# exie1122/micro-quad-SLAM

Measured on NVIDIA B200. Metric: ray_cell_updates_per_s, higher is better.
Workload: dtype i8

## Files before the change

micro-quad-slam_b200/csrc/uqs_api.cu:

```cuda
#include <algorithm>
#include <cmath>
#include <cstdarg>
#include <cstdio>
#include <cstring>
#include <vector>

#include "../../include/uqs_mapping.h"
#include "uqs_host.h"

namespace uqs {

static Context g_single;
Context* g_cur = &g_single;

static char g_err[512] = "";

void set_error(const char* fmt, ...) {
  va_list ap;
  va_start(ap, fmt);
  vsnprintf(g_err, sizeof(g_err), fmt, ap);
  va_end(ap);
}

int cuda_fail(cudaError_t e, const char* what) {
  set_error("CUDA error in %s: %s", what, cudaGetErrorString(e));
  return UQS_ERR_CUDA;
}

int DevBuf::ensure(size_t bytes) {
  if (bytes <= cap) return UQS_OK;
  if (p) cudaFree(p);
  p = nullptr;
  cap = 0;
  size_t want = bytes + bytes / 8 + 256;
  cudaError_t e = cudaMalloc(&p, want);
  if (e != cudaSuccess) {
    cudaGetLastError();
    want = bytes;
    e = cudaMalloc(&p, want);
  }
  if (e != cudaSuccess) {
    p = nullptr;
    set_error("cudaMalloc(%zu) failed: %s", want, cudaGetErrorString(e));
    return UQS_ERR_NOMEM;
  }
  cap = want;
  return UQS_OK;
}

void DevBuf::release() {
  if (p) cudaFree(p);
  p = nullptr;
  cap = 0;
}

int check_ready() {
  if (!g_ctx.ready) {
    if (!g_err[0]) set_error("uqs_init() has not been called or failed");
    return UQS_ERR_NOT_INIT;
  }
  return UQS_OK;
}

int make_dev_params(const uqs_params* p, DevParams* d) {
  if (!p) { set_error("params is NULL"); return UQS_ERR_BAD_ARG; }
  if (p->W < 2 || p->H < 2 || p->W > 32766 || p->H > 32766) {
    set_error("grid size %dx%d outside [2, 32766]", p->W, p->H);
    return UQS_ERR_BAD_ARG;
  }
  if (!(p->res_m > 0.0f) || !std::isfinite(p->origin_x) || !std::isfinite(p->origin_y)) {
    set_error("res_m must be > 0 and the origin finite");
    return UQS_ERR_BAD_ARG;
  }
  if (p->lo_min < -128 || p->lo_max > 127 || p->lo_min > p->lo_max) {
    set_error("log-odds clamp [%d,%d] does not fit int8", p->lo_min, p->lo_max);
    return UQS_ERR_BAD_ARG;
  }
  if (p->lo_free < 0 || p->lo_free > 127 || p->lo_occ < 0 || p->lo_occ > 127) {
    set_error("log-odds steps must be in [0,127]");
    return UQS_ERR_BAD_ARG;
  }
  d->W = p->W; d->H = p->H; d->halfW = p->W / 2; d->halfH = p->H / 2;
  d->res = p->res_m; d->ox = p->origin_x; d->oy = p->origin_y;
  d->max_range = p->max_range_m; d->min_range = p->min_range_m;
  volatile float mr = p->max_range_m, hm = p->hit_margin_m, fov = p->fov_deg;
  volatile float pi_f = (float)M_PI;
  d->hit_below = mr - hm;
  d->half_fov = fov * 0.5f;
  d->deg2rad = pi_f / 180.0f;
  for (int c = 0; c < 8; c++) {
    volatile float cf = (float)c;
    volatile float u = (cf - 3.5f) / 3.5f;
    volatile float hf = d->half_fov;
    d->col_off[c] = u * hf;
  }
  d->lo_free = p->lo_free; d->lo_occ = p->lo_occ; d->lo_min = p->lo_min; d->lo_max = p->lo_max;
  d->end_nohit = -(p->lo_free / 2);
  d->ranges_u16 = 0;
  return UQS_OK;
}

int ensure_inv_table() {
  if (g_ctx.inv_table.p) return UQS_OK;
  std::vector<uint32_t> t(kMaxRayCells + 1);
  t[0] = 0;
  for (uint32_t m = 1; m <= (uint32_t)kMaxRayCells; m++) t[m] = (uint32_t)(((1ull << 31) + m - 1) / m);
  int rc = g_ctx.inv_table.ensure(t.size() * sizeof(uint32_t));
  if (rc) return rc;
  cudaError_t e = cudaMemcpyAsync(g_ctx.inv_table.p, t.data(), t.size() * sizeof(uint32_t), cudaMemcpyHostToDevice, g_ctx.stream());
  if (e == cudaSuccess) e = cudaStreamSynchronize(g_ctx.stream());
  if (e == cudaSuccess) e = cudaDeviceSynchronize();
  if (e != cudaSuccess) { g_ctx.inv_table.release(); return cuda_fail(e, "inv table upload"); }
  return UQS_OK;
}

static void choose_tiles(int W, int rows, int target, int* sw, int* sh, int* nsx, int* nsy) {
  auto pick = [](int extent, int forced, int target, int* size, int* count) {
    if (forced > 0) {
      *size = std::min(forced, extent);
    } else {
      int n = std::max(1, (extent + target / 2) / target);
      int s = (extent + n - 1) / n;
      s = (s + 3) & ~3;
      *size = std::min(s, extent);
    }
    *count = (extent + *size - 1) / *size;
  };
  pick(W, g_ctx.tune_sw, target, sw, nsx);
  pick(rows, g_ctx.tune_sh, target >= 80 ? target + target / 4 : target, sh, nsy);
}

static cudaError_t zero_counted(void* p, size_t bytes, cudaStream_t st) {
  g_ctx.launches += bytes ? 1 : 0;
  return zero_async(p, bytes, st);
}

int replay_device(const DevParams& dp, int n_flights, int n_frames, const float* x, const float* y,
                  const float* yaw, const float* ranges, const uint8_t* kind, int8_t* grids,
                  int accumulate, int row0, int rows, bool reset_stats, const ProbeSet* probes) {
  cudaStream_t st = g_ctx.stream();
  const int gpf = (n_frames + 31) / 32;
  g_ctx.w->boxes_valid = false;
  {
    const int rc0 = ensure_inv_table();
    if (rc0) return rc0;
  }
  {
    const int side = std::max(dp.W, dp.H);
    const bool long_rays = side > kMaxRayCells + 1 && (kind != nullptr || !(dp.max_range / dp.res + 3.0f <= (float)kMaxRayCells));
    bool generic = g_ctx.engine == 3 || long_rays || dp.lo_min > 0 || dp.lo_max < 0;
    int rcg;
    if ((rcg = g_ctx.w->counters.ensure(64 * sizeof(unsigned long long)))) return rcg;
    unsigned long long* cnt = (unsigned long long*)g_ctx.w->counters.p;
    cudaError_t eg = cudaSuccess;
    if (!generic && accumulate) {
      unsigned long long bad = 0;
      eg = zero_counted(cnt + 40, sizeof(unsigned long long), st);
      if (eg == cudaSuccess) eg = range_check_launch(grids, n_flights, dp.W, dp.H, row0, rows, dp.lo_min, dp.lo_max, cnt + 40, st);
      if (eg == cudaSuccess) eg = cudaMemcpyAsync(&bad, cnt + 40, sizeof(bad), cudaMemcpyDeviceToHost, st);
      if (eg == cudaSuccess) eg = cudaStreamSynchronize(st);
      if (eg != cudaSuccess) return cuda_fail(eg, "start-grid range check");
      g_ctx.launches += 1;
      generic = bad != 0;
    }
    if (generic) {
      if (reset_stats) eg = zero_counted(cnt, 8 * sizeof(unsigned long long), st);
      if (eg != cudaSuccess) return cuda_fail(eg, "memset stats");
      ProbeArgs PA;
      if (probes && (rcg = probe_buckets(*probes, 0, n_flights, n_frames, dp.W, 0, 0, 0, 0, 0, 0, &PA))) return rcg;
      KernelTimer t_rep(2);
      eg = generic_launch(dp, n_flights, n_frames, x, y, yaw, ranges, kind, grids, accumulate, row0, rows, cnt, st, probes ? &PA : nullptr);
      t_rep.stop();
      if (eg != cudaSuccess) return cuda_fail(eg, "k_replay_generic launch");
      g_ctx.launches += accumulate ? 1 : 2;
      return UQS_OK;
    }
  }
  int sw, sh, nsx, nsy, slices = 1;
  choose_tiles(dp.W, rows, 80, &sw, &sh, &nsx, &nsy);
  {
    const long long warp_slots = (long long)g_ctx.sm_count * 32;
    const long long jobs80 = (long long)n_flights * nsx * nsy;
    int want = g_ctx.tune_slices;
    int slice_tile = 40;
    const bool band = rows < dp.H;
    if (want == 0 && band && g_ctx.tune_sw == 0 && g_ctx.tune_sh == 0 && jobs80 < 2 * warp_slots) {
      choose_tiles(dp.W, rows, 56, &sw, &sh, &nsx, &nsy);
      want = 1;
    }
    if (want == 0 && jobs80 < 2 * warp_slots) {
      const int s_max = std::max(1, std::min(64, gpf / 8));
      const bool long_rays = dp.max_range >= 200.0f * dp.res;
      long long jobs_t = 1;
      for (int t : { 56, 40, 24, 16 }) {
        if (t == 56 && !long_rays) continue;
        int a, b, nx, ny;
        choose_tiles(dp.W, rows, t, &a, &b, &nx, &ny);
        slice_tile = t;
        jobs_t = (long long)n_flights * nx * ny;
        if (jobs_t * s_max >= 8 * warp_slots) break;
      }
      want = (int)std::min<long long>(s_max, std::max<long long>(1, (16 * warp_slots + jobs_t - 1) / jobs_t));
    }
    if (want > 1) {
      const size_t map_bytes = (size_t)dp.W * dp.H * 4;
      const size_t cap = ((size_t)6 << 30) / map_bytes;
      want = (int)std::min<size_t>((size_t)want, std::max<size_t>(cap, 1) + 1);
    }
    if (want > 1) {
      slices = want;
      choose_tiles(dp.W, rows, slice_tile, &sw, &sh, &nsx, &nsy);
    }
  }
  int pitch = (sw + 3) & ~3;
  if (((pitch >> 2) & 1) == 0) pitch += 4;
  const int pitch_cells = sw | 1;
  if (slices > 1 && g_ctx.tune_slices == 0 && ((size_t)pitch_cells * sh * 4 + kReplayQueueBytes) * kReplayWarps > 227u * 1024u)
    slices = 1;
  const int gps = (gpf + slices - 1) / slices;
  const int tile_bytes = slices > 1 ? std::max(pitch * sh, pitch_cells * sh * 4) : pitch * sh;
  size_t smem = (size_t)tile_bytes * kReplayWarps + (size_t)kReplayQueueBytes * kReplayWarps;

  const int nw = g_ctx.flight_warps ? g_ctx.flight_warps
                 : ((n_flights >= 4 * g_ctx.sm_count || g_ctx.chip_shared) ? 4 : (n_flights >= 2 * g_ctx.sm_count ? 8 : 16));
  const bool may_reside = g_ctx.engine != 1 && row0 == 0 && rows == dp.H;
  if (g_ctx.engine == 2 && !may_reside) {
    set_error("engine 2 (resident) cannot replay a row band");
    return UQS_ERR_BAD_ARG;
  }
  if (smem > 227u * 1024u) {
    set_error("sub-tile %dx%d needs %zu B of shared memory per CTA (> 227 KB)", sw, sh, smem);
    return UQS_ERR_BAD_ARG;
  }

  const size_t per_flight = (size_t)n_frames * (32 * sizeof(uint2) + sizeof(uint4)) + (size_t)gpf * sizeof(uint2);
  const size_t budget = g_ctx.scratch_budget;
  int chunk = (int)std::max<size_t>(1, std::min<size_t>((size_t)n_flights, budget / std::max<size_t>(per_flight, 1)));
  chunk = std::min(chunk, 65535);
  int rc;
  if ((rc = g_ctx.w->rays.ensure((size_t)chunk * n_frames * 32 * sizeof(uint2)))) return rc;
  if ((rc = g_ctx.w->frames.ensure((size_t)chunk * n_frames * sizeof(uint4)))) return rc;
  if ((rc = g_ctx.w->groups.ensure((size_t)chunk * gpf * sizeof(uint2)))) return rc;
  if ((rc = g_ctx.w->counters.ensure(64 * sizeof(unsigned long long)))) return rc;
  unsigned long long* counters = (unsigned long long*)g_ctx.w->counters.p;
  cudaError_t e;
  if (reset_stats) {
    e = zero_counted(counters, 8 * sizeof(unsigned long long), st);
    if (e != cudaSuccess) return cuda_fail(e, "memset stats");
  }

  int ctas_per_sm = 0;
  e = tiles_prepare(probes != nullptr, smem, &ctas_per_sm);
  if (e != cudaSuccess) return cuda_fail(e, "occupancy(k_replay_tiles)");
  if (ctas_per_sm < 1) { set_error("replay kernel does not fit on an SM (smem %zu)", smem); return UQS_ERR_CUDA; }

  for (int f0 = 0; f0 < n_flights; f0 += chunk) {
    const int nf = std::min(chunk, n_flights - f0);
    const size_t fo = (size_t)f0 * n_frames;
    KernelTimer t_setup(1);
    k_ray_setup<<<dim3((unsigned)gpf, (unsigned)nf), 1024, 0, st>>>(
        dp, n_frames, x + fo, y + fo, yaw + fo,
        dp.ranges_u16 ? reinterpret_cast<const float*>(reinterpret_cast<const uint16_t*>(ranges) + fo * 32) : ranges + fo * 32,
        kind ? kind + fo : nullptr, may_reside ? 1 + g_ctx.k0_bias : 0,
        (const uint32_t*)g_ctx.inv_table.p, (uint4*)g_ctx.w->frames.p, (uint2*)g_ctx.w->groups.p, (uint2*)g_ctx.w->rays.p, counters);
    e = cudaGetLastError();
    t_setup.stop();
    if (e != cudaSuccess) return cuda_fail(e, "k_ray_setup launch");

    if (may_reside) {
      if ((rc = g_ctx.w->boxes.ensure((size_t)nf * sizeof(int4)))) return rc;
      int* d_dims = (int*)(counters + 32);
      if (!g_ctx.w->h_dims) {
        e = cudaHostAlloc((void**)&g_ctx.w->h_dims, 16, cudaHostAllocMapped);
        if (e != cudaSuccess) { g_ctx.w->h_dims = nullptr; return cuda_fail(e, "cudaHostAlloc(dims)"); }
      }
      int* h_dims_dev = nullptr;
      e = cudaHostGetDevicePointer((void**)&h_dims_dev, g_ctx.w->h_dims, 0);
      if (e == cudaSuccess) e = zero_counted(d_dims, 2 * sizeof(int), st);
      if (e == cudaSuccess)
        e = flight_boxes_launch(nf, gpf, (const uint2*)g_ctx.w->groups.p, dp.W, dp.H, (int4*)g_ctx.w->boxes.p, d_dims, h_dims_dev, st);
      if (e == cudaSuccess) e = cudaStreamSynchronize(st);
      if (e != cudaSuccess) return cuda_fail(e, "k_flight_boxes");
      const int dims[2] = { g_ctx.w->h_dims[0], g_ctx.w->h_dims[1] };
      g_ctx.launches += 2;
      g_ctx.w->boxes_valid = nf == n_flights;
      g_ctx.w->boxes_n = nf; g_ctx.w->box_w = dims[0]; g_ctx.w->box_h = dims[1];
      const int bw = std::max(dims[0], 4), bh = std::max(dims[1], 1);
      int fpitch = (bw + 3) & ~3;
      if (((fpitch >> 2) & 1) == 0) fpitch += 4;
      if (g_ctx.pitch_mod >= 0)
        while (((fpitch >> 2) & 31) != g_ctx.pitch_mod) fpitch += 4;
      const size_t region = (size_t)fpitch * bh;
      int ring_size = 256, f_ctas = 0, fnw = nw;
      size_t fsmem = 0;
      auto fit = [&](int w, int* ring, size_t* bytes, int* ctas) -> cudaError_t {
        *ring = 256;
        const size_t dec_bytes = (size_t)std::min(w, kDecSlotsMax) * kDecSlotBytes + 16;
        while (*ring > 32 && region + (size_t)(*ring + 4) * w + dec_bytes > kFlightSmemMax) *ring >>= 1;
        *bytes = region + (size_t)(*ring + 4) * w + dec_bytes;
        *ctas = 0;
        return *bytes <= kFlightSmemMax ? flights_prepare(w, g_ctx.flight_fan, g_ctx.flight_prod, *bytes, ctas) : cudaSuccess;
      };
      if (g_ctx.flight_warps) {
        e = fit(fnw, &ring_size, &fsmem, &f_ctas);
      } else {
        e = cudaSuccess;
        for (int w : { 4, 8, 16 }) {
          if (w < nw) continue;
          int r, c;
          size_t bts;
          if ((e = fit(w, &r, &bts, &c)) != cudaSuccess) break;
          if (c < 1) break;
          fnw = w; ring_size = r; fsmem = bts; f_ctas = c;
          if (c * w >= 24) break;
        }
      }
      if (e != cudaSuccess) return cuda_fail(e, "k_replay_flights attributes");
      if (g_ctx.engine == 2 && f_ctas < 1) {
        set_error("engine 2: the touched region %dx%d of a flight does not fit %zu B of shared memory", bw, bh, kFlightSmemMax);
        return UQS_ERR_BAD_ARG;
      }
      const bool pipelined = g_ctx.chip_shared;
      const bool resident = f_ctas >= 1 && (g_ctx.engine == 2 || nf * 4 >= g_ctx.sm_count || pipelined);
      if (resident) {
        FlightArgs FA;
        FA.frames = (const uint4*)g_ctx.w->frames.p;
        FA.rays = (const uint2*)g_ctx.w->rays.p;
        FA.boxes = (const int4*)g_ctx.w->boxes.p;
        FA.grids = grids + (size_t)f0 * dp.W * dp.H;
        FA.job_counter = counters + 8;
        FA.n_flights = nf; FA.n_frames = n_frames;
        FA.W = dp.W; FA.H = dp.H; FA.pitch = fpitch; FA.max_rows = bh; FA.ring_size = ring_size;
        FA.lo_free = dp.lo_free; FA.lo_occ = dp.lo_occ; FA.lo_min = dp.lo_min; FA.lo_max = dp.lo_max;
        FA.end_nohit = dp.end_nohit;
        FA.accumulate = accumulate;
        e = zero_counted(FA.job_counter, sizeof(unsigned long long), st);
        if (e == cudaSuccess && !accumulate) e = zero_counted(FA.grids, (size_t)nf * dp.W * dp.H, st);
        if (e != cudaSuccess) return cuda_fail(e, "memset before k_replay_flights");
        if (probes) {
          int p_ctas = 0;
          ProbeArgs PA;
          if ((rc = probe_buckets(*probes, f0, nf, n_frames, dp.W, 0, 0, 0, 0, 0, 0, &PA))) return rc;
          if ((e = flights_probe_prepare(fnw, fsmem, &p_ctas)) != cudaSuccess) return cuda_fail(e, "k_replay_flights (probes) attributes");
          if (p_ctas < 1) { set_error("resident engine (probes): %zu B of shared memory do not fit an SM", fsmem); return UQS_ERR_CUDA; }
          KernelTimer t_rep(2);
          e = flights_probe_launch(fnw, (unsigned)std::min<long long>(nf, (long long)p_ctas * g_ctx.sm_count), fsmem, st, FA, PA);
          t_rep.stop();
          if (e != cudaSuccess) return cuda_fail(e, "k_replay_flights (probes) launch");
          g_ctx.launches += 2;
          continue;
        }
        const unsigned fgrid = (unsigned)std::min<long long>(nf, (long long)f_ctas * g_ctx.sm_count);
        KernelTimer t_rep(2);
        e = flights_launch(fnw, g_ctx.flight_fan, g_ctx.flight_prod, fgrid, fsmem, st, FA);
        t_rep.stop();
        if (e != cudaSuccess) return cuda_fail(e, "k_replay_flights launch");
        g_ctx.launches += 2;
        continue;
      }
    }
    if (g_ctx.w->order_nsx != nsx || g_ctx.w->order_nsy != nsy) {
      std::vector<uint32_t> ord((size_t)nsx * nsy);
      for (uint32_t i = 0; i < ord.size(); i++) ord[i] = i;
      auto dist2 = [&](uint32_t t) {
        const double cx = ((t % nsx) + 0.5) * sw - dp.W * 0.5, cy = ((t / nsx) + 0.5) * sh + row0 - dp.H * 0.5;
        return cx * cx + cy * cy;
      };
      std::stable_sort(ord.begin(), ord.end(), [&](uint32_t a, uint32_t b) { return dist2(a) < dist2(b); });
      if ((rc = g_ctx.w->order.ensure(ord.size() * sizeof(uint32_t)))) return rc;
      e = cudaMemcpyAsync(g_ctx.w->order.p, ord.data(), ord.size() * sizeof(uint32_t), cudaMemcpyHostToDevice, st);
      if (e == cudaSuccess) e = cudaStreamSynchronize(st);
      if (e != cudaSuccess) return cuda_fail(e, "tile order upload");
      g_ctx.w->order_nsx = nsx;
      g_ctx.w->order_nsy = nsy;
    }
    ReplayArgs A;
    A.tile_order = (const uint32_t*)g_ctx.w->order.p;
    A.n_flights = nf;
    A.frames = (const uint4*)g_ctx.w->frames.p;
    A.groups = (const uint2*)g_ctx.w->groups.p;
    A.rays = (const uint2*)g_ctx.w->rays.p;
    A.grids = grids + (size_t)f0 * dp.W * dp.H;
    A.job_counter = counters + 8;
    A.total_jobs = (unsigned long long)nf * nsx * nsy * slices;
    A.slices = slices; A.groups_per_slice = gps; A.pitch_cells = pitch_cells;
    A.maps = nullptr;
    if (slices > 1) {
      if ((rc = g_ctx.w->maps.ensure((size_t)nf * (slices - 1) * dp.W * dp.H * sizeof(uint32_t)))) return rc;
      A.maps = (uint32_t*)g_ctx.w->maps.p;
    }
    A.n_frames = n_frames; A.groups_per_flight = gpf;
    A.W = dp.W; A.H = dp.H; A.row0 = row0; A.rows = rows;
    A.sw = sw; A.sh = sh; A.nsx = nsx; A.nsy = nsy;
    A.pitch = pitch; A.tile_bytes = tile_bytes;
    A.lo_free = dp.lo_free; A.lo_occ = dp.lo_occ; A.lo_min = dp.lo_min; A.lo_max = dp.lo_max;
    A.end_nohit = dp.end_nohit;
    A.accumulate = accumulate;
    e = zero_counted(A.job_counter, sizeof(unsigned long long), st);
    if (e != cudaSuccess) return cuda_fail(e, "memset job counter");
    unsigned long long want = (A.total_jobs + kReplayWarps - 1) / kReplayWarps;
    unsigned grid = (unsigned)std::min<unsigned long long>(want, (unsigned long long)ctas_per_sm * g_ctx.sm_count);
    ProbeArgs PA;
    if (probes && (rc = probe_buckets(*probes, f0, nf, n_frames, dp.W, slices, gps, sw, sh, nsx, nsy, &PA))) return rc;
    KernelTimer t_rep(2);
    e = tiles_launch(probes != nullptr, grid, smem, st, A, probes ? PA : ProbeArgs{});
    if (e == cudaSuccess && probes && slices > 1 &&
        (rc = probe_resolve_slices(PA, (int)probes->slots(), A.grids, A.maps, dp.W, dp.H, slices, gps)))
      return rc;
    if (e == cudaSuccess && slices > 1) {
      const size_t cells = (size_t)dp.W * rows * nf;
      k_compose_slices<<<(unsigned)((cells + 255) / 256), 256, 0, st>>>(A.grids, A.maps, nf, dp.W, dp.H, slices, row0, rows);
      e = cudaGetLastError();
      g_ctx.launches += 1;
    }
    t_rep.stop();
    if (e != cudaSuccess) return cuda_fail(e, "k_replay_tiles launch");
    g_ctx.launches += 2;
  }
  return UQS_OK;
}

int fetch_stats_mask(uqs_stats* stats, uint64_t frames, unsigned mask) {
  if (!stats) return UQS_OK;
  unsigned long long tot[4] = { 0, 0, 0, 0 };
  for (int i = 0; i < 3; i++) {
    if (!(mask & (1u << i)) || !g_ctx.works[i].counters.p) continue;
    Work* saved = g_ctx.w;
    g_ctx.w = &g_ctx.works[i];
    cudaStream_t st = g_ctx.stream();
    g_ctx.w = saved;
    unsigned long long h[4];
    cudaError_t e = cudaMemcpyAsync(h, g_ctx.works[i].counters.p, sizeof(h), cudaMemcpyDeviceToHost, st);
    if (e != cudaSuccess) return cuda_fail(e, "stats D2H");
    e = cudaStreamSynchronize(st);
    if (e != cudaSuccess) return cuda_fail(e, "stats sync");
    for (int k = 0; k < 4; k++) tot[k] += h[k];
  }
  stats->ray_cell_updates = tot[0];
  stats->rays_accepted = tot[1];
  stats->rays_skipped = tot[2];
  stats->domain_errors = tot[3];
  stats->frames = frames;
  if (tot[3]) {
    set_error("%llu rays longer than %d cells reached a fast engine (internal routing error)", tot[3], kMaxRayCells);
    return UQS_ERR_DOMAIN;
  }
  return UQS_OK;
}

int fetch_stats(uqs_stats* stats, uint64_t frames) { return fetch_stats_mask(stats, frames, 1u); }

int pose_device(int n_flights, int n_samples, const uint32_t* t_ms, const float* rx, const float* ry,
                const float* h, const float* yaw, const uint8_t* q, float* xo, float* yo, int mode) {
  cudaStream_t st = g_ctx.stream();
  const long long total = (long long)n_flights * n_samples;
  int rc;
  if ((rc = g_ctx.w->inc.ensure((size_t)total * 2 * sizeof(float)))) return rc;
  if ((rc = g_ctx.w->counters.ensure(64 * sizeof(unsigned long long)))) return rc;
  float* inc_n = (float*)g_ctx.w->inc.p;
  float* inc_e = inc_n + total;
  unsigned long long* dom = nullptr;
  cudaError_t e = cudaSuccess;
  volatile float pi_f = (float)M_PI;
  const float deg2rad = pi_f / 180.0f;
  KernelTimer t_pose(0);
  k_pose_increments<<<(unsigned)((total + 255) / 256), 256, 0, st>>>(total, n_samples, t_ms, rx, ry, h, yaw, q,
                                                                     deg2rad, inc_n, inc_e, dom);
  e = cudaGetLastError();
  if (e != cudaSuccess) return cuda_fail(e, "k_pose_increments launch");
  if (mode == 0) {
    const int warps_per_block = 4;
    k_pose_chain<<<(unsigned)((n_flights + warps_per_block - 1) / warps_per_block), warps_per_block * 32, 0, st>>>(
        n_flights, n_samples, inc_n, inc_e, xo, yo);
  } else {
    const int tile = pose_scan_tile();
    const int ppf = (n_samples + tile - 1) / tile;
    const size_t nparts = (size_t)n_flights * ppf;
    if ((rc = g_ctx.w->scan.ensure(nparts * pose_scan_state_bytes() + 64))) return rc;
    e = cudaMemsetAsync(g_ctx.w->scan.p, 0, nparts * pose_scan_state_bytes() + 64, st);
    if (e != cudaSuccess) return cuda_fail(e, "memset scan state");
    unsigned int* ticket = (unsigned int*)((char*)g_ctx.w->scan.p + nparts * pose_scan_state_bytes());
    k_pose_scan<<<(unsigned)nparts, pose_scan_threads(), 0, st>>>(n_flights, n_samples, ppf, inc_n, inc_e, xo, yo,
                                                                  (volatile ScanState*)g_ctx.w->scan.p, ticket);
  }
  e = cudaGetLastError();
  t_pose.stop();
  if (e != cudaSuccess) return cuda_fail(e, "pose kernel launch");
  g_ctx.launches += 2;
  return UQS_OK;
}

void context_select_single() {
  g_cur = &g_single;
  if (g_single.ready) cudaSetDevice(g_single.device);
}

int context_init(Context& c, int device) {
  int n = 0;
  cudaError_t e = cudaGetDeviceCount(&n);
  if (e != cudaSuccess || n <= 0) {
    cudaGetLastError();
    set_error("no CUDA device available (%s); this library has no CPU fallback",
              e != cudaSuccess ? cudaGetErrorString(e) : "device count is 0");
    c.ready = false;
    return UQS_ERR_NO_DEVICE;
  }
  if (device < 0 || device >= n) { set_error("device %d out of range (0..%d)", device, n - 1); return UQS_ERR_BAD_ARG; }
  if ((e = cudaSetDevice(device)) != cudaSuccess) return cuda_fail(e, "cudaSetDevice");
  cudaDeviceProp prop;
  if ((e = cudaGetDeviceProperties(&prop, device)) != cudaSuccess) return cuda_fail(e, "cudaGetDeviceProperties");
  if (prop.major < 10) {
    set_error("device %d is sm_%d%d; this library is built for sm_100a only", device, prop.major, prop.minor);
    return UQS_ERR_NO_DEVICE;
  }
  if ((e = cudaStreamCreateWithFlags(&c.own_stream, cudaStreamNonBlocking)) != cudaSuccess)
    return cuda_fail(e, "cudaStreamCreate");
  c.device = device;
  c.sm_count = prop.multiProcessorCount;
  c.ext_stream = nullptr;
  c.use_ext = false;
  c.ready = true;
  g_err[0] = 0;
  return UQS_OK;
}

void context_shutdown(Context& c) {
  if (!c.ready) return;
  cudaSetDevice(c.device);
  cudaDeviceSynchronize();
  comm_release();
  dropin_release();
  pipeline_release();
  c.release_all();
  if (c.own_stream) cudaStreamDestroy(c.own_stream);
  c.own_stream = nullptr;
  c.ready = false;
}

}

using namespace uqs;

extern "C" {

void uqs_params_default(uqs_params* p) {
  if (!p) return;
  p->W = 500; p->H = 500; p->res_m = 0.10f; p->size_m = 50.0f;
  p->origin_x = 0.0f; p->origin_y = 0.0f;
  p->max_range_m = 4.00f; p->fov_deg = 63.0f;
  p->min_range_m = 0.05f; p->hit_margin_m = 0.05f;
  p->lo_free = 1; p->lo_occ = 6; p->lo_min = -80; p->lo_max = 80;
}

const char* uqs_last_error(void) { return g_err; }

int uqs_init(int device) {
  g_cur = &g_single;
  if (g_single.ready && g_single.device == device) {
    cudaSetDevice(device);
    return UQS_OK;
  }
  if (g_single.ready) uqs_shutdown();
  return context_init(g_single, device);
}

void uqs_shutdown(void) {
  Context* saved = g_cur;
  g_cur = &g_single;
  context_shutdown(g_single);
  g_cur = (saved == &g_single) ? &g_single : saved;
}

int uqs_device_sm_count(void) { return g_ctx.ready ? g_ctx.sm_count : 0; }

int uqs_set_stream(void* s) {
  int rc = check_ready();
  if (rc) return rc;
  g_ctx.ext_stream = (cudaStream_t)s;
  g_ctx.use_ext = true;
  return UQS_OK;
}

int uqs_use_own_stream(void) {
  int rc = check_ready();
  if (rc) return rc;
  g_ctx.use_ext = false;
  return UQS_OK;
}

int uqs_sync(void) {
  int rc = check_ready();
  if (rc) return rc;
  cudaError_t e = cudaStreamSynchronize(g_ctx.stream());
  if (e != cudaSuccess) return cuda_fail(e, "cudaStreamSynchronize");
  return UQS_OK;
}

int uqs_set_tuning(int sw, int sh, int time_slices) {
  if (sw < 0 || sh < 0 || time_slices < 0) { set_error("negative tuning value"); return UQS_ERR_BAD_ARG; }
  g_ctx.tune_sw = sw;
  g_ctx.tune_sh = sh;
  g_ctx.tune_slices = time_slices;
  return UQS_OK;
}

int uqs_set_engine(int engine, int flight_warps) {
  if (engine < 0 || engine > 3 || (flight_warps != 0 && flight_warps != 4 && flight_warps != 8 && flight_warps != 16 && flight_warps != 32)) {
    set_error("engine must be 0 (auto), 1 (sub-tiles), 2 (grid resident) or 3 (unrestricted); warps 0, 4, 8, 16 or 32");
    return UQS_ERR_BAD_ARG;
  }
  g_ctx.engine = engine;
  g_ctx.flight_warps = flight_warps;
  return UQS_OK;
}

int uqs_set_resident_pitch_mod(int words_mod32) {
  g_ctx.pitch_mod = words_mod32 < 0 ? -1 : (words_mod32 & 31);
  return UQS_OK;
}

int uqs_set_decode_warp(int on) {
  g_ctx.flight_prod = on < 0 ? kDefaultDecodeWarp : (on ? 1 : 0);
  return UQS_OK;
}

int uqs_set_k0_bias(int steps) {
  g_ctx.k0_bias = steps < 0 ? 0 : (steps > 8 ? 8 : steps);
  return UQS_OK;
}

int uqs_set_fan_layout(int on) {
  g_ctx.flight_fan = on < 0 ? kDefaultFanLayout : (on ? 1 : 0);
  return UQS_OK;
}

unsigned long long uqs_kernel_launches(void) { return g_ctx.launches; }

int uqs_set_profiling(int on) {
  int rc = check_ready();
  if (rc) return rc;
  g_ctx.profiling = on != 0;
  return UQS_OK;
}

int uqs_profile_collect(double ms[3], int counts[3]) {
  int rc = check_ready();
  if (rc) return rc;
  cudaError_t e = cudaStreamSynchronize(g_ctx.stream());
  if (e != cudaSuccess) return cuda_fail(e, "profile sync");
  for (int i = 0; i < 3; i++) { ms[i] = 0.0; counts[i] = 0; }
  for (auto& s : g_ctx.spans) {
    float t = 0.f;
    if (s.kind < 3 && cudaEventElapsedTime(&t, s.a, s.b) == cudaSuccess) { ms[s.kind] += t; counts[s.kind]++; }
    cudaEventDestroy(s.a);
    cudaEventDestroy(s.b);
  }
  g_ctx.spans.clear();
  return UQS_OK;
}

int uqs_profile_timeline(double* out, int max_spans) {
  int rc = check_ready();
  if (rc) return -1;
  if (cudaDeviceSynchronize() != cudaSuccess || g_ctx.spans.empty() || !out) return 0;
  int n = 0;
  const cudaEvent_t ref = g_ctx.spans[0].a;
  for (auto& s : g_ctx.spans) {
    if (n >= max_spans) break;
    float t0 = 0.f, t1 = 0.f;
    if (cudaEventElapsedTime(&t0, ref, s.a) != cudaSuccess || cudaEventElapsedTime(&t1, ref, s.b) != cudaSuccess) continue;
    out[3 * n] = s.kind; out[3 * n + 1] = t0; out[3 * n + 2] = t1;
    n++;
  }
  return n;
}

int uqs_replay_dev(const uqs_params* p, int n_flights, int n_frames, const float* x, const float* y,
                   const float* yaw, const float* ranges, int8_t* grids, int accumulate, int row0,
                   int rows, uqs_stats* stats) {
  int rc = check_ready();
  if (rc) return rc;
  DevParams dp;
  if ((rc = make_dev_params(p, &dp))) return rc;
  if (n_flights <= 0 || n_frames <= 0 || !x || !y || !yaw || !ranges || !grids) {
    set_error("uqs_replay_dev: NULL pointer or non-positive size");
    return UQS_ERR_BAD_ARG;
  }
  if (row0 < 0 || rows <= 0 || row0 + rows > p->H) { set_error("row range [%d,%d) outside the grid", row0, row0 + rows); return UQS_ERR_BAD_ARG; }
  if ((rc = replay_device(dp, n_flights, n_frames, x, y, yaw, ranges, nullptr, grids, accumulate, row0, rows, true)))
    return rc;
  return fetch_stats(stats, (uint64_t)n_flights * n_frames);
}

int uqs_pose_integrate_dev(int n_flights, int n_samples, const uint32_t* t_ms, const float* rx,
                           const float* ry, const float* h, const float* yaw, const uint8_t* q,
                           float* xo, float* yo, int mode) {
  int rc = check_ready();
  if (rc) return rc;
  if (n_flights <= 0 || n_samples <= 0 || !t_ms || !rx || !ry || !h || !yaw || !q || !xo || !yo || (mode != 0 && mode != 1)) {
    set_error("uqs_pose_integrate_dev: bad argument");
    return UQS_ERR_BAD_ARG;
  }
  return pose_device(n_flights, n_samples, t_ms, rx, ry, h, yaw, q, xo, yo, mode);
}


static int h2d(DevBuf& b, const void* src, size_t bytes, const char* what) {
  int rc = b.ensure(bytes);
  if (rc) return rc;
  cudaError_t e = cudaMemcpyAsync(b.p, src, bytes, cudaMemcpyHostToDevice, g_ctx.stream());
  if (e != cudaSuccess) return cuda_fail(e, what);
  return UQS_OK;
}

int uqs_pose_integrate(int n_flights, int n_samples, const uint32_t* t_ms, const float* rx,
                       const float* ry, const float* h, const float* yaw, const uint8_t* q,
                       float* xo, float* yo, int mode) {
  int rc = check_ready();
  if (rc) return rc;
  if (n_flights <= 0 || n_samples <= 0 || !t_ms || !rx || !ry || !h || !yaw || !q || !xo || !yo || (mode != 0 && mode != 1)) {
    set_error("uqs_pose_integrate: bad argument");
    return UQS_ERR_BAD_ARG;
  }
  const size_t n = (size_t)n_flights * n_samples;
  if ((rc = h2d(g_ctx.in_t, t_ms, n * 4, "t_ms H2D"))) return rc;
  if ((rc = h2d(g_ctx.in_rx, rx, n * 4, "of_rate_x H2D"))) return rc;
  if ((rc = h2d(g_ctx.in_ry, ry, n * 4, "of_rate_y H2D"))) return rc;
  if ((rc = h2d(g_ctx.in_h, h, n * 4, "h_m H2D"))) return rc;
  if ((rc = h2d(g_ctx.in_yaw, yaw, n * 4, "yaw H2D"))) return rc;
  if ((rc = h2d(g_ctx.in_q, q, n, "of_q H2D"))) return rc;
  if ((rc = g_ctx.in_x.ensure(n * 4)) || (rc = g_ctx.in_y.ensure(n * 4))) return rc;
  if ((rc = pose_device(n_flights, n_samples, (uint32_t*)g_ctx.in_t.p, (float*)g_ctx.in_rx.p, (float*)g_ctx.in_ry.p,
                        (float*)g_ctx.in_h.p, (float*)g_ctx.in_yaw.p, (uint8_t*)g_ctx.in_q.p, (float*)g_ctx.in_x.p,
                        (float*)g_ctx.in_y.p, mode)))
    return rc;
  cudaError_t e = cudaMemcpyAsync(xo, g_ctx.in_x.p, n * 4, cudaMemcpyDeviceToHost, g_ctx.stream());
  if (e == cudaSuccess) e = cudaMemcpyAsync(yo, g_ctx.in_y.p, n * 4, cudaMemcpyDeviceToHost, g_ctx.stream());
  if (e == cudaSuccess) e = cudaStreamSynchronize(g_ctx.stream());
  if (e != cudaSuccess) return cuda_fail(e, "pose D2H");
  return UQS_OK;
}

int uqs_beam_cells(const uqs_params* p, int n_frames, const float* x, const float* y, const float* yaw,
                   const float* ranges, int32_t* cells_out, int32_t* origin_out) {
  int rc = check_ready();
  if (rc) return rc;
  DevParams dp;
  if ((rc = make_dev_params(p, &dp))) return rc;
  if (n_frames <= 0 || !x || !y || !yaw || !ranges || !cells_out || !origin_out) { set_error("uqs_beam_cells: bad argument"); return UQS_ERR_BAD_ARG; }
  if ((rc = ensure_inv_table())) return rc;
  cudaStream_t st = g_ctx.stream();
  const size_t n = (size_t)n_frames;
  const int gpf = (n_frames + 31) / 32;
  if ((rc = h2d(g_ctx.in_x, x, n * 4, "x H2D")) || (rc = h2d(g_ctx.in_y, y, n * 4, "y H2D")) ||
      (rc = h2d(g_ctx.in_yaw, yaw, n * 4, "yaw H2D")) || (rc = h2d(g_ctx.in_ranges, ranges, n * 128, "ranges H2D")))
    return rc;
  if ((rc = g_ctx.w->rays.ensure(n * 32 * sizeof(uint2))) || (rc = g_ctx.w->frames.ensure(n * sizeof(uint4))) ||
      (rc = g_ctx.w->groups.ensure((size_t)gpf * sizeof(uint2))) || (rc = g_ctx.w->counters.ensure(64 * 8)) ||
      (rc = g_ctx.out_grids.ensure(n * 32 * 2 * 4 + n * 2 * 4)))
    return rc;
  cudaError_t e = cudaMemsetAsync(g_ctx.w->counters.p, 0, 64, st);
  if (e != cudaSuccess) return cuda_fail(e, "memset");
  k_ray_setup<<<(unsigned)gpf, 1024, 0, st>>>(dp, n_frames, (float*)g_ctx.in_x.p, (float*)g_ctx.in_y.p,
                                              (float*)g_ctx.in_yaw.p, (float*)g_ctx.in_ranges.p, nullptr, 0,
                                              (const uint32_t*)g_ctx.inv_table.p, (uint4*)g_ctx.w->frames.p, (uint2*)g_ctx.w->groups.p,
                                              (uint2*)g_ctx.w->rays.p, (unsigned long long*)g_ctx.w->counters.p);
  int32_t* d_cells = (int32_t*)g_ctx.out_grids.p;
  int32_t* d_origin = d_cells + n * 64;
  k_records_to_cells<<<(unsigned)((n * 32 + 255) / 256), 256, 0, st>>>((long long)n, (uint4*)g_ctx.w->frames.p,
                                                                       (uint2*)g_ctx.w->rays.p, d_cells, d_origin);
  e = cudaGetLastError();
  if (e != cudaSuccess) return cuda_fail(e, "beam_cells kernels");
  e = cudaMemcpyAsync(cells_out, d_cells, n * 64 * 4, cudaMemcpyDeviceToHost, st);
  if (e == cudaSuccess) e = cudaMemcpyAsync(origin_out, d_origin, n * 2 * 4, cudaMemcpyDeviceToHost, st);
  if (e == cudaSuccess) e = cudaStreamSynchronize(st);
  if (e != cudaSuccess) return cuda_fail(e, "beam_cells D2H");
  g_ctx.launches += 2;
  return UQS_OK;
}

int uqs_frame_bounds(const uqs_params* p, int n_frames, const float* x, const float* y, const float* yaw,
                     const float* ranges, int32_t* k0_out, int32_t* sorted_out) {
  int rc = check_ready();
  if (rc) return rc;
  DevParams dp;
  if ((rc = make_dev_params(p, &dp))) return rc;
  if (n_frames <= 0 || !x || !y || !yaw || !ranges || !k0_out || !sorted_out) { set_error("uqs_frame_bounds: bad argument"); return UQS_ERR_BAD_ARG; }
  if ((rc = ensure_inv_table())) return rc;
  cudaStream_t st = g_ctx.stream();
  const size_t n = (size_t)n_frames;
  const int gpf = (n_frames + 31) / 32;
  if ((rc = h2d(g_ctx.in_x, x, n * 4, "x H2D")) || (rc = h2d(g_ctx.in_y, y, n * 4, "y H2D")) ||
      (rc = h2d(g_ctx.in_yaw, yaw, n * 4, "yaw H2D")) || (rc = h2d(g_ctx.in_ranges, ranges, n * 128, "ranges H2D")))
    return rc;
  if ((rc = g_ctx.w->rays.ensure(n * 32 * sizeof(uint2))) || (rc = g_ctx.w->frames.ensure(n * sizeof(uint4))) ||
      (rc = g_ctx.w->groups.ensure((size_t)gpf * sizeof(uint2))) || (rc = g_ctx.w->counters.ensure(64 * 8)))
    return rc;
  cudaError_t e = cudaMemsetAsync(g_ctx.w->counters.p, 0, 64, st);
  if (e != cudaSuccess) return cuda_fail(e, "memset");
  k_ray_setup<<<(unsigned)gpf, 1024, 0, st>>>(dp, n_frames, (float*)g_ctx.in_x.p, (float*)g_ctx.in_y.p,
                                              (float*)g_ctx.in_yaw.p, (float*)g_ctx.in_ranges.p, nullptr, 1,
                                              (const uint32_t*)g_ctx.inv_table.p, (uint4*)g_ctx.w->frames.p, (uint2*)g_ctx.w->groups.p,
                                              (uint2*)g_ctx.w->rays.p, (unsigned long long*)g_ctx.w->counters.p);
  e = cudaGetLastError();
  if (e != cudaSuccess) return cuda_fail(e, "k_ray_setup launch");
  std::vector<uint4> fr(n);
  e = cudaMemcpyAsync(fr.data(), g_ctx.w->frames.p, n * sizeof(uint4), cudaMemcpyDeviceToHost, st);
  if (e == cudaSuccess) e = cudaStreamSynchronize(st);
  if (e != cudaSuccess) return cuda_fail(e, "frame_bounds D2H");
  for (size_t i = 0; i < n; i++) {
    k0_out[i] = (fr[i].y & kFrameHasOrigin) ? (int32_t)(fr[i].x >> 16) : -1;
    sorted_out[i] = (fr[i].y & kFrameSorted) ? 1 : 0;
  }
  g_ctx.launches += 1;
  return UQS_OK;
}

int uqs_sincosf_batch(size_t n, const float* ang, float* s, float* c) {
  int rc = check_ready();
  if (rc) return rc;
  if (!n || !ang || !s || !c) { set_error("uqs_sincosf_batch: bad argument"); return UQS_ERR_BAD_ARG; }
  cudaStream_t st = g_ctx.stream();
  if ((rc = h2d(g_ctx.in_x, ang, n * 4, "ang H2D")) || (rc = g_ctx.in_y.ensure(n * 4)) || (rc = g_ctx.in_yaw.ensure(n * 4)))
    return rc;
  k_sincosf<<<(unsigned)((n + 255) / 256), 256, 0, st>>>(n, (float*)g_ctx.in_x.p, (float*)g_ctx.in_y.p, (float*)g_ctx.in_yaw.p);
  cudaError_t e = cudaGetLastError();
  if (e == cudaSuccess) e = cudaMemcpyAsync(s, g_ctx.in_y.p, n * 4, cudaMemcpyDeviceToHost, st);
  if (e == cudaSuccess) e = cudaMemcpyAsync(c, g_ctx.in_yaw.p, n * 4, cudaMemcpyDeviceToHost, st);
  if (e == cudaSuccess) e = cudaStreamSynchronize(st);
  if (e != cudaSuccess) return cuda_fail(e, "sincosf batch");
  g_ctx.launches += 1;
  return UQS_OK;
}

int uqs_measure_rmw_peak(double* updates_per_s) {
  int rc = check_ready();
  if (rc) return rc;
  if (!updates_per_s) { set_error("NULL output"); return UQS_ERR_BAD_ARG; }
  cudaStream_t st = g_ctx.stream();
  const int tile_bytes = 4096, iters = 8192;
  const size_t smem = (size_t)tile_bytes * kReplayWarps;
  cudaError_t e = cudaFuncSetAttribute(k_rmw_peak, cudaFuncAttributeMaxDynamicSharedMemorySize, (int)smem);
  if (e != cudaSuccess) return cuda_fail(e, "cudaFuncSetAttribute(k_rmw_peak)");
  int per_sm = 0;
  e = cudaOccupancyMaxActiveBlocksPerMultiprocessor(&per_sm, k_rmw_peak, kReplayThreads, smem);
  if (e != cudaSuccess || per_sm < 1) return cuda_fail(e, "occupancy(k_rmw_peak)");
  if ((rc = g_ctx.w->counters.ensure(64 * 8))) return rc;
  const unsigned grid = (unsigned)(per_sm * g_ctx.sm_count);
  cudaEvent_t a, b;
  cudaEventCreate(&a);
  cudaEventCreate(&b);
  k_rmw_peak<<<grid, kReplayThreads, smem, st>>>(tile_bytes, 64, -80, (int*)g_ctx.w->counters.p + 96);
  cudaEventRecord(a, st);
  k_rmw_peak<<<grid, kReplayThreads, smem, st>>>(tile_bytes, iters, -80, (int*)g_ctx.w->counters.p + 96);
  cudaEventRecord(b, st);
  e = cudaEventSynchronize(b);
  float ms = 0.f;
  cudaEventElapsedTime(&ms, a, b);
  cudaEventDestroy(a);
  cudaEventDestroy(b);
  if (e != cudaSuccess) return cuda_fail(e, "k_rmw_peak");
  const double updates = (double)grid * kReplayThreads * (double)iters * 8.0;
  *updates_per_s = updates / (ms * 1e-3);
  g_ctx.launches += 2;
  return UQS_OK;
}

int uqs_measure_atoms_peak(double* updates_per_s) {
  int rc = check_ready();
  if (rc) return rc;
  if (!updates_per_s) { set_error("NULL output"); return UQS_ERR_BAD_ARG; }
  cudaStream_t st = g_ctx.stream();
  const int tile_bytes = 4096, iters = 2048;
  const size_t smem = (size_t)tile_bytes * kReplayWarps;
  cudaError_t e = cudaFuncSetAttribute(k_atoms_peak, cudaFuncAttributeMaxDynamicSharedMemorySize, (int)smem);
  if (e != cudaSuccess) return cuda_fail(e, "cudaFuncSetAttribute(k_atoms_peak)");
  int per_sm = 0;
  e = cudaOccupancyMaxActiveBlocksPerMultiprocessor(&per_sm, k_atoms_peak, kReplayThreads, smem);
  if (e != cudaSuccess || per_sm < 1) return cuda_fail(e, "occupancy(k_atoms_peak)");
  if ((rc = g_ctx.w->counters.ensure(64 * 8))) return rc;
  const unsigned grid = (unsigned)(per_sm * g_ctx.sm_count);
  cudaEvent_t a, b;
  cudaEventCreate(&a);
  cudaEventCreate(&b);
  k_atoms_peak<<<grid, kReplayThreads, smem, st>>>(tile_bytes, 64, (int*)g_ctx.w->counters.p + 96);
  cudaEventRecord(a, st);
  k_atoms_peak<<<grid, kReplayThreads, smem, st>>>(tile_bytes, iters, (int*)g_ctx.w->counters.p + 96);
  cudaEventRecord(b, st);
  e = cudaEventSynchronize(b);
  float ms = 0.f;
  cudaEventElapsedTime(&ms, a, b);
  cudaEventDestroy(a);
  cudaEventDestroy(b);
  if (e != cudaSuccess) return cuda_fail(e, "k_atoms_peak");
  *updates_per_s = (double)grid * kReplayThreads * (double)iters * 8.0 / (ms * 1e-3);
  g_ctx.launches += 2;
  return UQS_OK;
}

}
```

micro-quad-slam_b200/csrc/uqs_device.cuh:

```cuda
#pragma once
#include <cstdint>
#include <cuda_runtime.h>

namespace uqs {

struct DevParams {
  int   W, H, halfW, halfH;
  float res, ox, oy;
  float max_range, min_range, hit_below;
  float half_fov;
  float col_off[8];
  float deg2rad;
  int   lo_free, lo_occ, lo_min, lo_max;
  int   end_nohit;
  int   ranges_u16;
};

__device__ __forceinline__ float range_from_mm(unsigned mm) {
  return mm == 0xFFFFu ? __int_as_float(0x7fc00000) : __fmul_rn((float)mm, 0.001f);
}

constexpr int      kMaxRayCells   = 1024;
constexpr uint32_t kRayHit        = 1u << 24;
constexpr uint32_t kRayValid      = 1u << 25;
constexpr uint32_t kFrameHasOrigin = 1u << 16;
constexpr uint32_t kFrameSorted    = 1u << 17;
constexpr uint32_t kEmptyBoxLoHi  = 0x00007fffu;

static __constant__ uint32_t kInvPio4[24] = {
  0xa2, 0xa2f9, 0xa2f983, 0xa2f9836e, 0xf9836e4e, 0x836e4e44, 0x6e4e4415, 0x4e441529, 0x441529fc, 0x1529fc27,
  0x29fc2757, 0xfc2757d1, 0x2757d1f5, 0x57d1f534, 0xd1f534dd, 0xf534ddc0, 0x34ddc0db, 0xddc0db62, 0xc0db6295,
  0xdb629599, 0x6295993c, 0x95993c43, 0x993c4390, 0x3c439041 };

__device__ __forceinline__ void sincosf_poly(double x, double xs, bool swap, bool neg_cos, float& sn, float& cs) {
  const double x2 = __dmul_rn(x, x);
  const double x3 = __dmul_rn(x2, xs);
  const double x4 = __dmul_rn(x2, x2);
  const double s1 = __fma_rn(x2, -0x1.994eb3774cf24p-13, 0x1.1107605230bc4p-7);
  const double c2 = __fma_rn(x2, 0x1.99343027bf8c3p-16, -0x1.6c087e89a359dp-10);
  const double c1 = __fma_rn(x2, -0x1.ffffffd0c621cp-2, 1.0);
  const double x5 = __dmul_rn(x2, x3);
  const double x6 = __dmul_rn(x2, x4);
  double S = __fma_rn(x3, -0x1.555545995a603p-3, xs);
  double C = __fma_rn(x4, 0x1.55553e1068f19p-5, c1);
  S = __fma_rn(x5, s1, S);
  C = __fma_rn(x6, c2, C);
  if (neg_cos) C = -C;
  const float fs = __double2float_rn(S), fc = __double2float_rn(C);
  if (swap) { cs = fs; sn = fc; } else { sn = fs; cs = fc; }
}

static __device__ __noinline__ void sincosf_large(float y, float& sn, float& cs) {
  uint32_t xi = __float_as_uint(y);
  if (((xi >> 20) & 0x7ffu) >= 0x7f8u) {
    const uint32_t nan = ((xi & 0x7fffffffu) == 0x7f800000u) ? 0xffc00000u : (xi | 0x00400000u);
    sn = cs = __uint_as_float(nan);
    return;
  }
  const int sign = (int)(xi >> 31);
  const uint32_t* arr = &kInvPio4[(xi >> 26) & 15u];
  const int shift = (int)((xi >> 23) & 7u);
  xi = ((xi & 0xffffffu) | 0x800000u) << shift;
  unsigned long long res0 = (unsigned long long)(uint32_t)(xi * arr[0]);
  const unsigned long long res1 = (unsigned long long)xi * arr[4];
  const unsigned long long res2 = (unsigned long long)xi * arr[8];
  res0 = (res2 >> 32) | (res0 << 32);
  res0 += res1;
  const unsigned long long nn = (res0 + (1ull << 61)) >> 62;
  res0 -= nn << 62;
  const double x = __dmul_rn(__ll2double_rn((long long)res0), 0x1.921FB54442D18p-62);
  const int n = (int)nn;
  const double xs = (((n + sign) + 1) & 2) ? -x : x;
  sincosf_poly(x, xs, (n & 1) != 0, ((n + sign) & 2) != 0, sn, cs);
}

__device__ __forceinline__ bool sincosf_glibc(float y, float& sn, float& cs) {
  const uint32_t top12 = (__float_as_uint(y) >> 20) & 0x7ffu;
  if (top12 >= 0x42fu) {
    sincosf_large(y, sn, cs);
    return true;
  }
  double x = (double)y;
  const double r = __dmul_rn(x, 0x1.45f306dc9c883p+23);
  const int n = (__double2int_rz(r) + 0x800000) >> 24;
  x = __fma_rn(-(double)n, 0x1.921fb54442d18p+0, x);
  const double xs = ((n + 1) & 2) ? -x : x;
  const double x2 = __dmul_rn(x, x);
  const double x3 = __dmul_rn(x2, xs);
  const double x4 = __dmul_rn(x2, x2);
  const double s1 = __fma_rn(x2, -0x1.994eb3774cf24p-13, 0x1.1107605230bc4p-7);
  const double c2 = __fma_rn(x2, 0x1.99343027bf8c3p-16, -0x1.6c087e89a359dp-10);
  const double c1 = __fma_rn(x2, -0x1.ffffffd0c621cp-2, 1.0);
  const double x5 = __dmul_rn(x2, x3);
  const double x6 = __dmul_rn(x2, x4);
  double S = __fma_rn(x3, -0x1.555545995a603p-3, xs);
  double C = __fma_rn(x4, 0x1.55553e1068f19p-5, c1);
  S = __fma_rn(x5, s1, S);
  C = __fma_rn(x6, c2, C);
  if (n & 2) C = -C;
  const float fs = __double2float_rn(S), fc = __double2float_rn(C);
  const bool tiny = top12 < 0x398u;
  if (n & 1) { cs = fs; sn = fc; } else { sn = fs; cs = fc; }
  if (tiny) { sn = y; cs = 1.0f; }
  return true;
}

__device__ __forceinline__ int lrintf_as_int(float q) {
  if (fabsf(q) < 2147483520.0f) return __float2int_rn(q);
  const long long r = (fabsf(q) < 9223372036854775808.0f) ? __float2ll_rn(q)
                                                          : (long long)0x8000000000000000ull;
  return (int)r;
}

__device__ __forceinline__ bool world_to_grid(const DevParams& p, float wx, float wy, int& gx,
                                              int& gy) {
  const float ddx = __fsub_rn(wx, p.ox);
  const float ddy = __fsub_rn(wy, p.oy);
  const int ix = (int)((unsigned)lrintf_as_int(__fdiv_rn(ddx, p.res)) + (unsigned)p.halfW);
  const int iy = (int)((unsigned)lrintf_as_int(__fdiv_rn(ddy, p.res)) + (unsigned)p.halfH);
  gx = ix;
  gy = iy;
  return !(ix < 0 || ix >= p.W || iy < 0 || iy >= p.H);
}

__device__ __forceinline__ int beam_endpoint(const DevParams& p, float px, float py, float yaw_deg,
                                             float dist, int b, float& ex, float& ey, bool& hit) {
  if (isnan(dist)) return 0;
  if (dist <= p.min_range) return 0;
  hit = dist < p.hit_below;
  if (dist > p.max_range) dist = p.max_range;
  const int d = b >> 3, c = b & 7;
  const float centre = (d & 1) ? ((d & 2) ? -90.0f : 90.0f) : ((d & 2) ? 180.0f : 0.0f);
  const float off = p.col_off[c];
  const float ang_deg = __fadd_rn(__fadd_rn(yaw_deg, centre), off);
  const float ang = __fmul_rn(ang_deg, p.deg2rad);
  float sn, cs;
  if (!sincosf_glibc(ang, sn, cs)) return -1;
  ex = __fadd_rn(px, __fmul_rn(dist, cs));
  ey = __fadd_rn(py, __fmul_rn(dist, sn));
  return 1;
}

__device__ __forceinline__ int sext12(uint32_t v) { return ((int)(v << 20)) >> 20; }

__device__ __forceinline__ float frontier_ray_angle(const DevParams& p, float yaw_deg, float offset_deg, int r) {
  const float ro = (r == 0) ? 0.0f : (r == 1) ? 15.0f : -15.0f;
  return __fmul_rn(__fadd_rn(__fadd_rn(yaw_deg, offset_deg), ro), p.deg2rad);
}
__device__ __forceinline__ float frontier_step(const DevParams& p) { return __fmul_rn(p.res, 2.0f); }
constexpr float kFrontierRange = 2.5f;
__device__ __forceinline__ bool frontier_point(const DevParams& p, float x, float y, float d, float ca, float sa, int& gx,
                                               int& gy) {
  const float px = __fadd_rn(x, __fmul_rn(d, ca));
  const float py = __fadd_rn(y, __fmul_rn(d, sa));
  return world_to_grid(p, px, py, gx, gy);
}
__device__ __forceinline__ int frontier_weight(int v) {
  return (v >= -1 && v <= 1) ? 3 : (v > 10) ? -4 : (v < -10) ? 1 : 0;
}

__device__ __forceinline__ int minor_steps(int k, int n2, int h2, uint32_t inv) {
  return (int)__umulhi((uint32_t)(k * n2 + h2), inv);
}

}
```

micro-quad-slam_b200/csrc/uqs_host.h:

```cpp
#pragma once
#include <cstddef>
#include <cstdint>
#include <cuda_runtime.h>
#include <vector>

#include "../../include/uqs_mapping.h"
#include "uqs_kernels.cuh"

namespace uqs {

constexpr int kDefaultDecodeWarp = 0;
constexpr int kDefaultFanLayout = 0;

struct DevBuf {
  void* p = nullptr;
  size_t cap = 0;
  int ensure(size_t bytes);
  void release();
};

struct Work {
  DevBuf rays, frames, groups, counters, inc, scan, order, maps, boxes;
  DevBuf probe_slots, probe_keys, probe_sorted, probe_start, probe_tmp;
  int order_nsx = 0, order_nsy = 0;
  cudaStream_t stream = nullptr;
  int* h_dims = nullptr;
  bool boxes_valid = false;
  int boxes_n = 0, box_w = 0, box_h = 0;
  void release() {
    if (h_dims) cudaFreeHost(h_dims);
    h_dims = nullptr;
    DevBuf* all[] = { &rays, &frames, &groups, &counters, &inc, &scan, &order, &maps, &boxes, &probe_slots, &probe_keys, &probe_sorted,
                      &probe_start, &probe_tmp };
    order_nsx = order_nsy = 0;
    for (DevBuf* b : all) b->release();
  }
};

struct Context {
  bool ready = false;
  int device = -1;
  int sm_count = 0;
  cudaStream_t own_stream = nullptr;
  cudaStream_t ext_stream = nullptr;
  bool use_ext = false;
  int tune_sw = 0, tune_sh = 0, tune_slices = 0;
  int engine = 0;
  int flight_warps = 0;
  int k0_bias = 0;
  int pitch_mod = -1;
  int flight_prod = kDefaultDecodeWarp;
  int flight_fan = kDefaultFanLayout;
  int host_chunk = 0;
  bool copy_only = false;
  bool chip_shared = false;
  size_t scratch_budget = (size_t)12 << 30;
  unsigned long long launches = 0;
  DevBuf inv_table;
  Work works[3];
  Work* w = &works[0];
  DevBuf in_t, in_rx, in_ry, in_h, in_yaw, in_q, in_x, in_y, in_ranges, in_kind, out_grids;
  void* pipeline = nullptr;
  void* comm = nullptr;
  int comm_rank = 0, comm_nranks = 1;
  int band_edges[17] = { 0 };

  bool profiling = false;
  struct Span { cudaEvent_t a, b; int kind; };
  std::vector<Span> spans;

  cudaStream_t stream() const { return w->stream ? w->stream : (use_ext ? ext_stream : own_stream); }
  cudaStream_t user_stream() const { return use_ext ? ext_stream : own_stream; }
  void release_all() {
    DevBuf* all[] = { &in_t, &in_rx, &in_ry, &in_h, &in_yaw, &in_q, &in_x, &in_y, &in_ranges, &in_kind, &out_grids };
    for (DevBuf* b : all) b->release();
    for (Work& k : works) k.release();
    inv_table.release();
  }
};

constexpr size_t kFlightSmemMax = 227u * 1024u - 64u;

extern Context* g_cur;
#define g_ctx (*::uqs::g_cur)
int context_init(Context& c, int device);
void context_shutdown(Context& c);
void context_select_single();

void set_error(const char* fmt, ...);
int cuda_fail(cudaError_t e, const char* what);
int check_ready();
int make_dev_params(const uqs_params* p, DevParams* d);
struct ProbeSet {
  int n_queries = 0, s_max = 0;
  const uqs_query* queries = nullptr;
  const int* cells = nullptr;
  uint32_t* values = nullptr;
  size_t slots() const { return (size_t)n_queries * 3 * s_max; }
};
int probe_buckets(const ProbeSet& Q, int f0, int nf, int n_frames, int W, int slices, int groups_per_slice, int sw,
                  int sh, int nsx, int nsy, ProbeArgs* out);
int probe_resolve_slices(const ProbeArgs& A, int n_probes_max, const int8_t* grids, const uint32_t* maps, int W, int H,
                         int slices, int groups_per_slice);

int replay_device(const DevParams& dp, int n_flights, int n_frames, const float* x, const float* y,
                  const float* yaw, const float* ranges, const uint8_t* kind, int8_t* grids,
                  int accumulate, int row0, int rows, bool reset_stats, const ProbeSet* probes = nullptr);
int fetch_stats(uqs_stats* stats, uint64_t frames);
int ensure_inv_table();
cudaError_t generic_launch(const DevParams& dp, int n_flights, int n_frames, const float* x, const float* y, const float* yaw,
                           const float* ranges, const uint8_t* kind, int8_t* grids, int accumulate, int row0, int rows,
                           unsigned long long* stats, cudaStream_t st, const ProbeArgs* Q = nullptr);
cudaError_t range_check_launch(const int8_t* grids, int n_flights, int W, int H, int row0, int rows, int lo_min, int lo_max,
                               unsigned long long* bad, cudaStream_t st);
int fetch_stats_mask(uqs_stats* stats, uint64_t frames, unsigned mask);
void dropin_release();
void pipeline_release();
void comm_release();
int pose_device(int n_flights, int n_samples, const uint32_t* t_ms, const float* rx, const float* ry,
                const float* h, const float* yaw, const uint8_t* q, float* xo, float* yo, int mode);

struct KernelTimer {
  int kind;
  cudaStream_t st;
  cudaEvent_t a = nullptr, b = nullptr;
  explicit KernelTimer(int k, cudaStream_t on = nullptr) : kind(k), st(on ? on : g_ctx.stream()) {
    if (g_ctx.profiling && cudaEventCreate(&a) == cudaSuccess && cudaEventCreate(&b) == cudaSuccess)
      cudaEventRecord(a, st);
  }
  void stop() {
    if (a && b) {
      cudaEventRecord(b, st);
      g_ctx.spans.push_back({a, b, kind});
    }
  }
};

}
```

micro-quad-slam_b200/csrc/uqs_kernels.cu:

```cuda
#include <algorithm>
#include <cstdio>

#include "uqs_kernels.cuh"

namespace uqs {


__global__ void k_pose_increments(long long total, int n_samples, const uint32_t* __restrict__ t_ms,
                                  const float* __restrict__ rate_x, const float* __restrict__ rate_y,
                                  const float* __restrict__ h_m, const float* __restrict__ yaw_deg,
                                  const uint8_t* __restrict__ q, float deg2rad,
                                  float* __restrict__ inc_n, float* __restrict__ inc_e,
                                  unsigned long long* __restrict__ ) {
  const long long i = (long long)blockIdx.x * blockDim.x + threadIdx.x;
  if (i >= total) return;
  const int s = (int)(i % n_samples);
  float dn = 0.0f, de = 0.0f;
  if (s > 0) {
    const float rx = rate_x[i], ry = rate_y[i], h = h_m[i], yw = yaw_deg[i];
    if (q[i] >= 50 && !isnan(rx) && !isnan(ry) && !isnan(h) && !isnan(yw)) {
      const float dt = __fmul_rn((float)(t_ms[i] - t_ms[i - 1]), 0.001f);
      const float vbx = __fmul_rn(rx, h);
      const float vby = __fmul_rn(ry, h);
      const float a = __fmul_rn(yw, deg2rad);
      float sn, cs;
      sincosf_glibc(a, sn, cs);
      const float vn = __fsub_rn(__fmul_rn(vbx, cs), __fmul_rn(vby, sn));
      const float ve = __fadd_rn(__fmul_rn(vbx, sn), __fmul_rn(vby, cs));
      dn = __fmul_rn(vn, dt);
      de = __fmul_rn(ve, dt);
    }
  }
  inc_n[i] = dn;
  inc_e[i] = de;
}

constexpr int kChainChunk = 256;
constexpr int kChainWarps = 4;

__global__ void __launch_bounds__(kChainWarps * 32)
k_pose_chain(int n_flights, int n_samples, const float* __restrict__ inc_n,
             const float* __restrict__ inc_e, float* __restrict__ xo,
             float* __restrict__ yo) {
  __shared__ __align__(16) float s_n[kChainWarps][kChainChunk], s_e[kChainWarps][kChainChunk];
  const int wib = threadIdx.x >> 5, lane = threadIdx.x & 31;
  const int flight = blockIdx.x * kChainWarps + wib;
  if (flight >= n_flights) return;
  const size_t base = (size_t)flight * n_samples;
  float* sn = s_n[wib];
  float* se = s_e[wib];
  constexpr int PER = kChainChunk / 32;
  float rn[PER], re[PER];
  auto fetch = [&](int s0) {
#pragma unroll
    for (int u = 0; u < PER; u++) {
      const int s = s0 + u * 32 + lane;
      rn[u] = (s < n_samples) ? __ldg(&inc_n[base + s]) : 0.0f;
      re[u] = (s < n_samples) ? __ldg(&inc_e[base + s]) : 0.0f;
    }
  };
  fetch(0);
  float px = 0.0f, py = 0.0f;
  for (int s0 = 0; s0 < n_samples; s0 += kChainChunk) {
#pragma unroll
    for (int u = 0; u < PER; u++) { sn[u * 32 + lane] = rn[u]; se[u * 32 + lane] = re[u]; }
    if (s0 + kChainChunk < n_samples) fetch(s0 + kChainChunk);
    __syncwarp();
    if (lane == 0) {
      const float4* vn = reinterpret_cast<const float4*>(sn);
      const float4* ve = reinterpret_cast<const float4*>(se);
      float4 a0 = vn[0], b0 = ve[0], a1 = vn[1], b1 = ve[1];
#pragma unroll 4
      for (int g = 0; g < kChainChunk / 4; g++) {
        const int gn = min(g + 2, kChainChunk / 4 - 1);
        const float4 a2 = vn[gn], b2 = ve[gn];
        float4 a = a0, b = b0;
        a.x = px = __fadd_rn(px, a.x); b.x = py = __fadd_rn(py, b.x);
        a.y = px = __fadd_rn(px, a.y); b.y = py = __fadd_rn(py, b.y);
        a.z = px = __fadd_rn(px, a.z); b.z = py = __fadd_rn(py, b.z);
        a.w = px = __fadd_rn(px, a.w); b.w = py = __fadd_rn(py, b.w);
        reinterpret_cast<float4*>(sn)[g] = a;
        reinterpret_cast<float4*>(se)[g] = b;
        a0 = a1; b0 = b1; a1 = a2; b1 = b2;
      }
    }
    __syncwarp();
#pragma unroll
    for (int u = 0; u < PER; u++) {
      const int s = s0 + u * 32 + lane;
      if (s < n_samples) { xo[base + s] = sn[u * 32 + lane]; yo[base + s] = se[u * 32 + lane]; }
    }
    __syncwarp();
  }
}

constexpr int kScanThreads = 256;
constexpr int kScanItems = 8;
constexpr int kScanTile = kScanThreads * kScanItems;

struct ScanState { double agg_n, agg_e, inc_n, inc_e; int flag; int pad; };

__global__ void __launch_bounds__(kScanThreads)
k_pose_scan(int n_flights, int n_samples, int parts_per_flight, const float* __restrict__ inc_n,
            const float* __restrict__ inc_e, float* __restrict__ xo, float* __restrict__ yo,
            volatile ScanState* state, unsigned int* ticket) {
  __shared__ unsigned int s_part;
  __shared__ double s_wn[kScanThreads / 32], s_we[kScanThreads / 32];
  __shared__ double s_prefix_n, s_prefix_e;
  if (threadIdx.x == 0) s_part = atomicAdd(ticket, 1u);
  __syncthreads();
  const unsigned int part = s_part;
  if (part >= (unsigned)(n_flights * parts_per_flight)) return;
  const int flight = part / parts_per_flight, pf = part % parts_per_flight;
  const size_t base = (size_t)flight * n_samples;
  const int s_begin = pf * kScanTile + threadIdx.x * kScanItems;

  double vn[kScanItems], ve[kScanItems];
  double tn = 0.0, te = 0.0;
#pragma unroll
  for (int k = 0; k < kScanItems; k++) {
    const int s = s_begin + k;
    const double a = (s < n_samples) ? (double)inc_n[base + s] : 0.0;
    const double b = (s < n_samples) ? (double)inc_e[base + s] : 0.0;
    tn += a; te += b;
    vn[k] = tn; ve[k] = te;
  }
  const int lane = threadIdx.x & 31, wid = threadIdx.x >> 5;
  double wn = tn, we = te;
#pragma unroll
  for (int o = 1; o < 32; o <<= 1) {
    const double un = __shfl_up_sync(0xffffffffu, wn, o), ue = __shfl_up_sync(0xffffffffu, we, o);
    if (lane >= o) { wn += un; we += ue; }
  }
  if (lane == 31) { s_wn[wid] = wn; s_we[wid] = we; }
  __syncthreads();
  double off_n = 0.0, off_e = 0.0;
  for (int w = 0; w < wid; w++) { off_n += s_wn[w]; off_e += s_we[w]; }
  const double excl_n = off_n + wn - tn, excl_e = off_e + we - te;

  if (threadIdx.x == kScanThreads - 1) {
    const double agg_n = off_n + wn, agg_e = off_e + we;
    double pre_n = 0.0, pre_e = 0.0;
    if (pf == 0) {
      state[part].inc_n = agg_n; state[part].inc_e = agg_e;
      __threadfence();
      state[part].flag = 2;
    } else {
      state[part].agg_n = agg_n; state[part].agg_e = agg_e;
      __threadfence();
      state[part].flag = 1;
      int p = (int)part - 1;
      for (;;) {
        int f;
        while ((f = state[p].flag) == 0) { }
        __threadfence();
        if (f == 2) { pre_n += state[p].inc_n; pre_e += state[p].inc_e; break; }
        pre_n += state[p].agg_n; pre_e += state[p].agg_e;
        p--;
      }
      state[part].inc_n = pre_n + agg_n; state[part].inc_e = pre_e + agg_e;
      __threadfence();
      state[part].flag = 2;
    }
    s_prefix_n = pre_n; s_prefix_e = pre_e;
  }
  __syncthreads();
  const double bn = s_prefix_n + excl_n, be = s_prefix_e + excl_e;
#pragma unroll
  for (int k = 0; k < kScanItems; k++) {
    const int s = s_begin + k;
    if (s < n_samples) {
      xo[base + s] = (float)(bn + vn[k]);
      yo[base + s] = (float)(be + ve[k]);
    }
  }
}

int pose_scan_tile() { return kScanTile; }
int pose_scan_threads() { return kScanThreads; }
size_t pose_scan_state_bytes() { return sizeof(ScanState); }

__device__ __forceinline__ void mbar_init(uint32_t bar, uint32_t count) {
  asm volatile("mbarrier.init.shared::cta.b64 [%0], %1;" ::"r"(bar), "r"(count) : "memory");
  asm volatile("fence.mbarrier_init.release.cluster;" ::: "memory");
  asm volatile("fence.proxy.async.shared::cta;" ::: "memory");
}
__device__ __forceinline__ void bulk_load_g2s(uint32_t dst, const void* src, uint32_t bytes, uint32_t bar) {
  asm volatile("mbarrier.arrive.expect_tx.shared::cta.b64 _, [%0], %1;" ::"r"(bar), "r"(bytes) : "memory");
  asm volatile("cp.async.bulk.shared::cluster.global.mbarrier::complete_tx::bytes [%0], [%1], %2, [%3];" ::"r"(dst), "l"(src),
               "r"(bytes), "r"(bar)
               : "memory");
}
__device__ __forceinline__ void mbar_wait(uint32_t bar, uint32_t parity) {
  asm volatile(
      "{\n"
      ".reg .pred p;\n"
      "UQS_WAIT:\n"
      "mbarrier.try_wait.parity.shared::cta.b64 p, [%0], %1;\n"
      "@!p bra UQS_WAIT;\n"
      "}\n" ::"r"(bar),
      "r"(parity)
      : "memory");
}

__global__ void __launch_bounds__(1024, 2)
k_ray_setup(const __grid_constant__ DevParams p, int n_frames, const float* __restrict__ x,
            const float* __restrict__ y, const float* __restrict__ yaw_deg,
            const float* __restrict__ ranges, const uint8_t* __restrict__ kind, int want_k0,
            const uint32_t* __restrict__ inv_table, uint4* __restrict__ frames, uint2* __restrict__ groups, uint2* __restrict__ rays,
            unsigned long long* __restrict__ stats ) {
  __shared__ __align__(128) float s_rng[32 * 32];
  __shared__ __align__(8) unsigned long long s_bar;
  __shared__ int s_box[4][32];
  __shared__ unsigned s_cnt[2][32];
  __shared__ int s_org[32][2];
  const int lane = threadIdx.x & 31, w = threadIdx.x >> 5;
  const int flight = blockIdx.y, g = blockIdx.x, groups_per_flight = gridDim.x;
  const int f = g * 32 + w;
  const size_t fbase = (size_t)flight * n_frames;
  const int nfr = min(32, n_frames - g * 32);

  const bool u16 = p.ranges_u16 != 0;
  const unsigned rbytes = u16 ? 64u : 128u;
  const unsigned char* ranges_b = reinterpret_cast<const unsigned char*>(ranges);
  const unsigned char* blk_ranges = ranges_b + (fbase + (size_t)g * 32) * rbytes;
  const bool staged = (reinterpret_cast<size_t>(ranges) & 15) == 0;
  const uint32_t bar_sa = (uint32_t)__cvta_generic_to_shared(&s_bar);
  if (staged) {
    if (threadIdx.x == 0) {
      mbar_init(bar_sa, 1);
      bulk_load_g2s((uint32_t)__cvta_generic_to_shared(s_rng), blk_ranges, (uint32_t)nfr * rbytes, bar_sa);
    }
    __syncthreads();
  }

  int xmin = 0x7fff, xmax = 0, ymin = 0x7fff, ymax = 0;
  unsigned cells = 0;
  int accepted = 0, skipped = 0, domain = 0;

  if (w == 31) {
    int ox = -1, oy = -1;
    const int fo = g * 32 + lane;
    if (fo < n_frames && !world_to_grid(p, x[fbase + fo], y[fbase + fo], ox, oy)) ox = oy = -1;
    s_org[lane][0] = ox;
    s_org[lane][1] = oy;
  }

  const bool live = f < n_frames;
  const size_t fi = fbase + (live ? f : 0);
  float ex = 0.f, ey = 0.f;
  bool hit = false, raw = false;
  int st = 0;
  if (live) {
    const float px = x[fi], py = y[fi], third = yaw_deg[fi];
    raw = kind != nullptr && kind[fi] == 1;
    if (staged) mbar_wait(bar_sa, 0);
    const unsigned char* rb = staged ? reinterpret_cast<const unsigned char*>(s_rng) + (size_t)w * rbytes : ranges_b + fi * rbytes;
    const float* rr = reinterpret_cast<const float*>(rb);
    if (!raw) {
      const float dist = u16 ? range_from_mm(reinterpret_cast<const uint16_t*>(rb)[lane]) : rr[lane];
      st = beam_endpoint(p, px, py, third, dist, lane, ex, ey, hit);
    } else {
      st = (lane == 0) ? 1 : 0;
      ex = third;
      ey = rr[0];
      hit = rr[1] != 0.0f;
    }
  }
  __syncthreads();

  if (live) {
    const int gx0 = s_org[w][0], gy0 = s_org[w][1];
    const bool have_o = gx0 >= 0;
    uint32_t w0 = 0, w1 = 0;
    if (st < 0) {
      domain = 1;
    } else if (st > 0 && have_o) {
      int gx1, gy1;
      if (world_to_grid(p, ex, ey, gx1, gy1)) {
        const int dx = gx1 - gx0, dy = gy1 - gy0;
        const int m = max(abs(dx), abs(dy));
        if (m > kMaxRayCells) {
          domain = 1;
        } else {
          w0 = ((uint32_t)dx & 0xfffu) | (((uint32_t)dy & 0xfffu) << 12) | (hit ? kRayHit : 0u) |
               kRayValid;
          w1 = __ldg(&inv_table[m]);
          xmin = min(gx0, gx1); xmax = max(gx0, gx1);
          ymin = min(gy0, gy1); ymax = max(gy0, gy1);
          cells = (unsigned)m + 1u;
          accepted = 1;
        }
      }
    }
    if (!accepted && !domain && !(raw && lane != 0)) skipped = 1;
    rays[fi * 32 + lane] = make_uint2(w0, w1);

    int k0 = 0;
    bool frame_sorted = false;
    if (want_k0) {
      const int dx = sext12(w0), dy = sext12(w0 >> 12);
      const int adx = abs(dx), ady = abs(dy);
      const bool xmaj = adx >= ady;
      const int m = accepted ? (xmaj ? adx : ady) : -1;
      const int n = xmaj ? ady : adx;
      const bool xpos = dx >= 0, ypos = dy >= 0;
      float ra, rb;
      if (xmaj) { ra = xpos ? (ypos ? 0.f : 8.f) : 4.f; rb = (xpos == ypos) ? 1.f : -1.f; }
      else      { ra = ypos ? 2.f : 6.f;                rb = (xpos == ypos) ? -1.f : 1.f; }
      float sigma = (m > 0) ? ra + rb * __fdividef((float)n, (float)m) : 0.f;
      if (sigma >= 8.f) sigma -= 8.f;
      const int mmax = __reduce_max_sync(0xffffffffu, m);
      const unsigned any = __ballot_sync(0xffffffffu, m >= 0);
      const unsigned dir = __ballot_sync(0xffffffffu, m >= 1);
      const unsigned above = dir & ~(0xffffffffu >> (31 - lane));
      const int nxt = above ? (__ffs(above) - 1) : (__ffs(dir) - 1);
      const float sn = __shfl_sync(0xffffffffu, sigma, nxt & 31);
      const bool has_dir = m >= 1;
      float gap = sn - sigma;
      int A = (int)ra, sgn_n = (rb > 0.f) ? n : -n;
      if (A == 8 && n == 0) A = 0;
      const int pk = (A << 24) | ((sgn_n & 0xfff) << 12) | (max(m, 0) & 0xfff);
      const int pn = __shfl_sync(0xffffffffu, pk, nxt & 31);
      const int A2 = pn >> 24, n2s = (pn << 8) >> 20, m2 = pn & 0xfff;
      const int order = (A2 - A) * m * m2 + n2s * m - sgn_n * m2;
      const bool wraps = has_dir && order < 0;
      if (order == 0) gap = 0.f;
      else if (order < 0) gap += 8.f;
      gap = fmaxf(gap, 0.f);
      const bool sorted = __popc(__ballot_sync(0xffffffffu, wraps)) <= 1;
      frame_sorted = sorted;
      if (__popc(any) >= 2) {
        if (sorted || __popc(dir) < 2) {
          int kk = 1;
          if (has_dir && __popc(dir) >= 2) kk = (gap > 1e-4f) ? (int)(1.0f / (gap - 2e-5f)) + 1 : 0x7fffffff;
          k0 = min(__reduce_max_sync(0xffffffffu, kk) + (want_k0 - 1), mmax + 1);
        } else {
#pragma unroll 4
          for (int j = 1; j <= 16; j++) {
            const int pl = (lane + j) & 31;
            const float sp = __shfl_sync(0xffffffffu, sigma, pl);
            const int mp = __shfl_sync(0xffffffffu, m, pl);
            float dlt = fabsf(sigma - sp);
            dlt = fminf(dlt, 8.f - dlt);
            int kk = (dlt > 1e-4f) ? (int)(1.0f / (dlt - 2e-5f)) + 1 : 0x7fffffff;
            if (m < 1 || mp < 1) kk = 1;
            kk = min(kk, min(m, mp) + 1);
            if (m >= 0 && mp >= 0) k0 = max(k0, kk);
          }
          k0 = __reduce_max_sync(0xffffffffu, k0);
        }
      }
    }

    xmin = __reduce_min_sync(0xffffffffu, xmin);
    xmax = __reduce_max_sync(0xffffffffu, xmax);
    ymin = __reduce_min_sync(0xffffffffu, ymin);
    ymax = __reduce_max_sync(0xffffffffu, ymax);
    if (lane == 0)
      frames[fi] = make_uint4(have_o ? ((uint32_t)gx0 | ((uint32_t)k0 << 16)) : 0u,
                              have_o ? ((uint32_t)gy0 | kFrameHasOrigin | (frame_sorted ? kFrameSorted : 0u)) : 0u,
                              (uint32_t)xmin | ((uint32_t)xmax << 16),
                              (uint32_t)ymin | ((uint32_t)ymax << 16));
  }
  const unsigned as = __reduce_add_sync(0xffffffffu, (unsigned)accepted | ((unsigned)skipped << 16));
  const unsigned cd = __reduce_add_sync(0xffffffffu, cells | ((unsigned)domain << 21));
  if (lane == 0) {
    s_box[0][w] = xmin; s_box[1][w] = xmax; s_box[2][w] = ymin; s_box[3][w] = ymax;
    s_cnt[0][w] = as; s_cnt[1][w] = cd;
  }
  __syncthreads();
  if (w == 0) {
    const int bx0 = __reduce_min_sync(0xffffffffu, s_box[0][lane]);
    const int bx1 = __reduce_max_sync(0xffffffffu, s_box[1][lane]);
    const int by0 = __reduce_min_sync(0xffffffffu, s_box[2][lane]);
    const int by1 = __reduce_max_sync(0xffffffffu, s_box[3][lane]);
    const unsigned bas = __reduce_add_sync(0xffffffffu, s_cnt[0][lane]);
    const unsigned long long bcd = s_cnt[1][lane];
    const unsigned bc = __reduce_add_sync(0xffffffffu, (unsigned)(bcd & 0x1fffffu));
    const unsigned bd = __reduce_add_sync(0xffffffffu, (unsigned)(bcd >> 21));
    if (lane == 0)
      groups[(size_t)flight * groups_per_flight + g] =
          make_uint2((uint32_t)bx0 | ((uint32_t)bx1 << 16), (uint32_t)by0 | ((uint32_t)by1 << 16));
    if (lane < 4) {
      const unsigned long long t = lane == 0 ? bc : (lane == 1 ? (bas & 0xffffu) : (lane == 2 ? (bas >> 16) : bd));
      if (t) atomicAdd(&stats[lane], t);
    }
  }
}

__global__ void k_records_to_cells(long long n_frames, const uint4* __restrict__ frames,
                                   const uint2* __restrict__ rays, int32_t* __restrict__ cells,
                                   int32_t* __restrict__ origin) {
  const long long i = (long long)blockIdx.x * blockDim.x + threadIdx.x;
  if (i >= n_frames * 32) return;
  const long long f = i >> 5;
  const uint4 fr = frames[f];
  const uint2 r = rays[i];
  int cx = -1, cy = -1;
  if (r.x & kRayValid) {
    cx = (int)(fr.x & 0xffffu) + sext12(r.x);
    cy = (int)(fr.y & 0xffffu) + sext12(r.x >> 12);
  }
  cells[2 * i] = cx;
  cells[2 * i + 1] = cy;
  if ((i & 31) == 0) {
    origin[2 * f] = (fr.y & kFrameHasOrigin) ? (int)(fr.x & 0xffffu) : -1;
    origin[2 * f + 1] = (fr.y & kFrameHasOrigin) ? (int)(fr.y & 0xffffu) : -1;
  }
}

__global__ void k_sincosf(size_t n, const float* __restrict__ a, float* __restrict__ s,
                          float* __restrict__ c) {
  const size_t i = (size_t)blockIdx.x * blockDim.x + threadIdx.x;
  if (i >= n) return;
  float sn, cs;
  sincosf_glibc(a[i], sn, cs);
  s[i] = sn;
  c[i] = cs;
}

__global__ void k_world_to_grid_one(DevParams p, float wx, float wy, int* out ) {
  int gx, gy;
  const bool ok = world_to_grid(p, wx, wy, gx, gy);
  out[0] = ok ? 1 : 0;
  out[1] = gx;
  out[2] = gy;
}


__device__ __forceinline__ bool box_overlaps(uint32_t xlohi, uint32_t ylohi, int X0, int X1, int Y0,
                                             int Y1) {
  const int bx0 = (int)(xlohi & 0xffffu), bx1 = (int)(xlohi >> 16);
  const int by0 = (int)(ylohi & 0xffffu), by1 = (int)(ylohi >> 16);
  return bx0 < X1 && bx1 >= X0 && by0 < Y1 && by1 >= Y0;
}

struct SmemRegion { uint32_t lo, hi; };
#ifdef UQS_DEBUG_BOUNDS
__device__ __noinline__ void uqs_bounds_fail(uint32_t a, uint32_t n, uint32_t lo, uint32_t hi, int line) {
  printf("UQS_DEBUG_BOUNDS: shared access [%u, %u) outside region [%u, %u) at uqs_kernels.cu:%d (block %d thread %d)\n", a, a + n,
         lo, hi, line, (int)blockIdx.x, (int)threadIdx.x);
  __trap();
}
#define UQS_CHECK(a, n, R) do { const uint32_t a_ = (a); if (a_ < (R).lo || a_ + (n) > (R).hi) uqs_bounds_fail(a_, (n), (R).lo, (R).hi, __LINE__); } while (0)
#else
#define UQS_CHECK(a, n, R) ((void)0)
#endif

__device__ __forceinline__ int lds_s8(uint32_t a) {
  int v;
  asm volatile("ld.shared.s8 %0, [%1];" : "=r"(v) : "r"(a) : "memory");
  return v;
}
__device__ __forceinline__ void sts_u8(uint32_t a, int v) {
  asm volatile("st.shared.u8 [%0], %1;" ::"r"(a), "r"(v) : "memory");
}
__device__ __forceinline__ uint32_t lds_u32(uint32_t a) {
  uint32_t v;
  asm volatile("ld.shared.u32 %0, [%1];" : "=r"(v) : "r"(a) : "memory");
  return v;
}
__device__ __forceinline__ void sts_u32(uint32_t a, uint32_t v) {
  asm volatile("st.shared.u32 [%0], %1;" ::"r"(a), "r"(v) : "memory");
}
__device__ __forceinline__ uint4 lds_v4(uint32_t a) {
  uint4 v;
  asm volatile("ld.shared.v4.u32 {%0,%1,%2,%3}, [%4];" : "=r"(v.x), "=r"(v.y), "=r"(v.z), "=r"(v.w) : "r"(a) : "memory");
  return v;
}
__device__ __forceinline__ void sts_v4(uint32_t a, uint32_t x, uint32_t y, uint32_t z, uint32_t w) {
  asm volatile("st.shared.v4.u32 [%0], {%1,%2,%3,%4};" ::"r"(a), "r"(x), "r"(y), "r"(z), "r"(w) : "memory");
}
__device__ __forceinline__ int in_reg(int v) {
  asm volatile("" : "+r"(v));
  return v;
}


struct TileConsts { int pitch, lo_free, lo_occ, lo_min, lo_max, end_nohit; };
struct TileRegions { SmemRegion tile, queue; };

__device__ __forceinline__ int div_small(int num, int den) {
  int q = (int)((float)num * __frcp_rn((float)den));
  const int r = num - q * den;
  q += (r >= den) ? 1 : 0;
  q -= (r < 0) ? 1 : 0;
  return q;
}

constexpr int kQueueEntries = 64;
constexpr int kQueueBytes = kQueueEntries * 12;
static_assert(kQueueBytes == kReplayQueueBytes, "the host sizes the queues");

template <bool MAP>
__device__ __forceinline__ void apply_queued(const TileConsts& A, const TileRegions& DR, uint32_t tile, int lane, uint32_t queue, int head,
                                             int count, int X0, int X1, int Y0, int Y1) {
  (void)DR;
  uint32_t p1, p2, p3, p4, inv_l;
  bool live;
  {
    const uint32_t at = queue + 4u * (uint32_t)((head + lane) & (kQueueEntries - 1));
    UQS_CHECK(at, 4u, DR.queue); UQS_CHECK(at + 8u * kQueueEntries, 4u, DR.queue);
    const uint32_t w0 = lds_u32(at), org = lds_u32(at + 8u * kQueueEntries);
    inv_l = lds_u32(at + 4u * kQueueEntries);
    const int gx0 = (int)(org & 0xffffu), gy0 = (int)(org >> 16);
    const int dx = sext12(w0), dy = sext12(w0 >> 12);
    const int adx = abs(dx), ady = abs(dy);
    const bool xmaj = adx >= ady;
    const int m = xmaj ? adx : ady, n = xmaj ? ady : adx, h = m >> 1;
    const bool majpos = (xmaj ? dx : dy) >= 0, minpos = (xmaj ? dy : dx) >= 0;
    const int c0 = xmaj ? gx0 : gy0, c1 = xmaj ? gy0 : gx0;
    const int A0 = xmaj ? X0 : Y0, A1 = xmaj ? X1 : Y1;
    const int B0 = xmaj ? Y0 : X0, B1 = xmaj ? Y1 : X1;
    int ka = max(majpos ? (A0 - c0) : (c0 - (A1 - 1)), 0);
    int kb = min(majpos ? (A1 - 1 - c0) : (c0 - A0), m);
    const int qlo = minpos ? (B0 - c1) : (c1 - (B1 - 1));
    const int qhi = minpos ? (B1 - 1 - c1) : (c1 - B0);
    live = lane < count && qhi >= 0 && qlo <= n;
    if (qlo > 0 && qlo <= n) {
      const int num = qlo * m - h;
      ka = max(ka, div_small(num + n - 1, n));
    }
    if (qhi >= 0 && qhi < n) kb = min(kb, div_small((qhi + 1) * m - h - 1, n));
    live = live && ka <= kb;
    const int pitch = A.pitch;
    const int cK = majpos ? (xmaj ? 1 : pitch) : (xmaj ? -1 : -pitch);
    const int cQ = minpos ? (xmaj ? pitch : 1) : (xmaj ? -pitch : -1);
    p1 = (uint32_t)(2 * n) | ((uint32_t)m << 16);
    p2 = ((uint32_t)cK & 0xffffu) | ((uint32_t)cQ << 16);
    p3 = (uint32_t)ka | ((uint32_t)kb << 11) | ((w0 & kRayHit) ? (1u << 22) : 0u);
    p4 = tile + ((uint32_t)((gy0 - Y0) * pitch + (gx0 - X0)) << (MAP ? 2 : 0));
  }
  unsigned active = __ballot_sync(0xffffffffu, live);
  while (active) {
    const int b = __ffs(active) - 1;
    active &= active - 1;
    const uint32_t inv = __shfl_sync(0xffffffffu, inv_l, b);
    const uint32_t q1 = __shfl_sync(0xffffffffu, p1, b);
    const uint32_t q2 = __shfl_sync(0xffffffffu, p2, b);
    const uint32_t q3 = __shfl_sync(0xffffffffu, p3, b);
    const uint32_t base = __shfl_sync(0xffffffffu, p4, b);
    const int n2 = (int)(q1 & 0xffffu), m = (int)(q1 >> 16), h2 = m & ~1;
    const int cK = (int)(short)(q2 & 0xffffu), cQ = (int)q2 >> 16;
    const int k1 = (int)((q3 >> 11) & 0x7ffu);
    const int end_delta = (q3 & (1u << 22)) ? A.lo_occ : A.end_nohit;
    for (int k = (int)(q3 & 0x7ffu) + lane; k <= k1; k += 32) {
      const int q = minor_steps(k, n2, h2, inv);
      const int delta = (k == m) ? end_delta : -A.lo_free;
      if (!MAP) {
        const uint32_t cell = base + (uint32_t)(k * cK + q * cQ);
        UQS_CHECK(cell, 1u, DR.tile);
        const int v = lds_s8(cell) + delta;
        sts_u8(cell, min(max(v, A.lo_min), A.lo_max));
      } else {
        const uint32_t cell = base + ((uint32_t)(k * cK + q * cQ) << 2);
        UQS_CHECK(cell, 4u, DR.tile);
        const uint32_t w = lds_u32(cell);
        int flo = (int)(int8_t)(w & 0xffu), fhi = (int)(int8_t)((w >> 8) & 0xffu), a = (int)w >> 16;
        flo = min(max(flo + delta, A.lo_min), A.lo_max);
        fhi = min(max(fhi + delta, A.lo_min), A.lo_max);
        a = min(max(a + delta, -30000), 30000);
        sts_u32(cell, ((uint32_t)flo & 0xffu) | (((uint32_t)fhi & 0xffu) << 8) | ((uint32_t)a << 16));
      }
    }
    __syncwarp();
  }
}

extern __shared__ __align__(16) unsigned char uqs_smem[];

template <bool PROBE>
__global__ void __launch_bounds__(kReplayThreads)
k_replay_tiles(ReplayArgs A, ProbeArgs Q) {
  const int lane = threadIdx.x & 31;
  const int wic = threadIdx.x >> 5;
  int8_t* tile = reinterpret_cast<int8_t*>(uqs_smem) + (size_t)wic * A.tile_bytes;
  const uint32_t tile_s = (uint32_t)__cvta_generic_to_shared(tile);
  const uint32_t queue_s = (uint32_t)__cvta_generic_to_shared(uqs_smem) + (uint32_t)(kReplayWarps * A.tile_bytes + wic * kQueueBytes);
  const int lo_free = in_reg(A.lo_free), lo_occ = in_reg(A.lo_occ), lo_min = in_reg(A.lo_min), lo_max = in_reg(A.lo_max);
  const TileConsts CV = { in_reg(A.pitch), lo_free, lo_occ, lo_min, lo_max, in_reg(A.end_nohit) };
  const TileConsts CM = { in_reg(A.pitch_cells), lo_free, lo_occ, lo_min, lo_max, CV.end_nohit };
  const int subs_per_grid = A.nsx * A.nsy;
  const int S = A.slices;

  for (;;) {
    unsigned long long job = 0;
    if (lane == 0) job = atomicAdd(A.job_counter, 1ull);
    job = __shfl_sync(0xffffffffu, job, 0);
    if (job >= A.total_jobs) break;
    const unsigned long long per_group = (unsigned long long)kJobGroup * subs_per_grid * S;
    const int grp = (int)(job / per_group);
    const int in_grp = (int)(job - (unsigned long long)grp * per_group);
    const int gsize = min(kJobGroup, A.n_flights - grp * kJobGroup);
    const int flight = grp * kJobGroup + in_grp % gsize;
    const int rank = in_grp / gsize;
    const int slice = rank % S;
    const int sub = A.tile_order ? (int)A.tile_order[rank / S] : rank / S;
    const int X0 = (sub % A.nsx) * A.sw, Y0 = A.row0 + (sub / A.nsx) * A.sh;
    const int X1 = min(X0 + A.sw, A.W), Y1 = min(Y0 + A.sh, A.row0 + A.rows);
    const int tw = X1 - X0, th = Y1 - Y0;
    int8_t* grid = A.grids + (size_t)flight * A.W * A.H;
    const bool vec = ((A.W | X0 | tw) & 3) == 0 && ((reinterpret_cast<size_t>(grid) & 3) == 0);
    const bool map = slice > 0;
    TileRegions DR;
    DR.tile.lo = tile_s;
    DR.tile.hi = tile_s + (uint32_t)(map ? A.pitch_cells * th * 4 : A.pitch * th);
    DR.queue.lo = queue_s;
    DR.queue.hi = queue_s + (uint32_t)kQueueBytes;
    (void)DR;

    if (map) {
      const uint32_t ident = ((uint32_t)lo_min & 0xffu) | (((uint32_t)lo_max & 0xffu) << 8);
      for (int i = lane; i < A.pitch_cells * th; i += 32) reinterpret_cast<uint32_t*>(tile)[i] = ident;
    } else if (A.accumulate) {
      if (vec) {
        const int wpr = tw >> 2;
        for (int i = lane; i < wpr * th; i += 32) {
          const int r = i / wpr, c = i - r * wpr;
          *reinterpret_cast<uint32_t*>(tile + r * A.pitch + 4 * c) =
              *reinterpret_cast<const uint32_t*>(grid + (size_t)(Y0 + r) * A.W + X0 + 4 * c);
        }
      } else {
        for (int i = lane; i < tw * th; i += 32) {
          const int r = i / tw, c = i - r * tw;
          tile[r * A.pitch + c] = grid[(size_t)(Y0 + r) * A.W + X0 + c];
        }
      }
    } else {
      for (int i = lane; i < (A.pitch >> 2) * th; i += 32) reinterpret_cast<uint32_t*>(tile)[i] = 0u;
    }
    __syncwarp();

    const uint2* groups = A.groups + (size_t)flight * A.groups_per_flight;
    const uint4* frames = A.frames + (size_t)flight * A.n_frames;
    const uint2* rays = A.rays + (size_t)flight * A.n_frames * 32;
    const int g_begin = slice * A.groups_per_slice;
    const int g_end = min(g_begin + A.groups_per_slice, A.groups_per_flight);
    int qhead = 0, qn = 0;
    auto flush = [&]() {
      const int count = min(qn, 32);
      __syncwarp();
      if (map) apply_queued<true>(CM, DR, tile_s, lane, queue_s, qhead, count, X0, X1, Y0, Y1);
      else     apply_queued<false>(CV, DR, tile_s, lane, queue_s, qhead, count, X0, X1, Y0, Y1);
      qhead = (qhead + count) & (kQueueEntries - 1);
      qn -= count;
    };
    int pb = 0, pe = 0, next_pf = 0x7fffffff;
    if (PROBE) {
      const int b = (flight * S + slice) * subs_per_grid + sub;
      pb = Q.start[b];
      pe = Q.start[b + 1];
      if (pb < pe) next_pf = Q.probes[pb].x;
    }
    auto serve = [&](int fmax) {
      if (next_pf >= fmax) return;
      while (qn > 0) flush();
      __syncwarp();
      while (next_pf < fmax) {
        const int i = pb + lane;
        const int4 pr = i < pe ? Q.probes[i] : make_int4(0x7fffffff, 0, 0, 0);
        const bool take = pr.x < fmax;
        if (take) {
          const int gy = pr.y / A.W, gx = pr.y - gy * A.W;
          uint32_t v;
          if (map) {
            const uint32_t cell = tile_s + ((uint32_t)((gy - Y0) * A.pitch_cells + (gx - X0)) << 2);
            UQS_CHECK(cell, 4u, DR.tile);
            v = lds_u32(cell);
          } else {
            const uint32_t cell = tile_s + (uint32_t)((gy - Y0) * A.pitch + (gx - X0));
            UQS_CHECK(cell, 1u, DR.tile);
            v = (uint32_t)lds_s8(cell);
          }
          Q.values[pr.z] = v;
        }
        pb += __popc(__ballot_sync(0xffffffffu, take));
        next_pf = pb < pe ? Q.probes[pb].x : 0x7fffffff;
      }
    };
    for (int g0 = g_begin; g0 < g_end; g0 += 32) {
      bool ghit = false;
      if (g0 + lane < g_end) {
        const uint2 gb = __ldg(&groups[g0 + lane]);
        ghit = box_overlaps(gb.x, gb.y, X0, X1, Y0, Y1);
      }
      unsigned gmask = __ballot_sync(0xffffffffu, ghit);
      while (gmask) {
        const int gi = __ffs(gmask) - 1;
        gmask &= gmask - 1;
        const int f0 = (g0 + gi) * 32;
        uint4 fr = make_uint4(0, 0, kEmptyBoxLoHi, kEmptyBoxLoHi);
        if (f0 + lane < A.n_frames) fr = __ldg(&frames[f0 + lane]);
        unsigned fmask = __ballot_sync(0xffffffffu, box_overlaps(fr.z, fr.w, X0, X1, Y0, Y1));
        uint2 rec_next = make_uint2(0, 0);
        if (fmask) rec_next = __ldg(&rays[(size_t)(f0 + __ffs(fmask) - 1) * 32 + lane]);
        while (fmask) {
          const int fi = __ffs(fmask) - 1;
          fmask &= fmask - 1;
          const uint2 rec = rec_next;
          if (fmask) rec_next = __ldg(&rays[(size_t)(f0 + __ffs(fmask) - 1) * 32 + lane]);
          if (PROBE) serve(f0 + fi);
          const int gx0 = (int)(__shfl_sync(0xffffffffu, fr.x, fi) & 0xffffu);
          const int gy0 = (int)(__shfl_sync(0xffffffffu, fr.y, fi) & 0xffffu);
          const int ex = gx0 + sext12(rec.x), ey = gy0 + sext12(rec.x >> 12);
          const bool near = (rec.x & kRayValid) != 0u && min(gx0, ex) < X1 && max(gx0, ex) >= X0 && min(gy0, ey) < Y1 &&
                            max(gy0, ey) >= Y0;
          const unsigned nm = __ballot_sync(0xffffffffu, near);
          if (nm == 0u) continue;
          if (near) {
            const uint32_t at = queue_s + 4u * (uint32_t)((qhead + qn + __popc(nm & ((1u << lane) - 1u))) & (kQueueEntries - 1));
            UQS_CHECK(at, 4u, DR.queue); UQS_CHECK(at + 8u * kQueueEntries, 4u, DR.queue);
            sts_u32(at, rec.x);
            sts_u32(at + 4u * kQueueEntries, rec.y);
            sts_u32(at + 8u * kQueueEntries, (uint32_t)gx0 | ((uint32_t)gy0 << 16));
          }
          qn += __popc(nm);
          if (qn >= 32) flush();
        }
      }
    }
    while (qn > 0) flush();
    __syncwarp();
    if (PROBE) serve(0x7fffffff);

    if (map) {
      uint32_t* out = A.maps + ((size_t)flight * (S - 1) + (slice - 1)) * A.W * A.H;
      for (int i = lane; i < tw * th; i += 32) {
        const int r = i / tw, c = i - r * tw;
        out[(size_t)(Y0 + r) * A.W + X0 + c] = reinterpret_cast<const uint32_t*>(tile)[r * A.pitch_cells + c];
      }
    } else if (vec) {
      const int wpr = tw >> 2;
      for (int i = lane; i < wpr * th; i += 32) {
        const int r = i / wpr, c = i - r * wpr;
        *reinterpret_cast<uint32_t*>(grid + (size_t)(Y0 + r) * A.W + X0 + 4 * c) =
            *reinterpret_cast<const uint32_t*>(tile + r * A.pitch + 4 * c);
      }
    } else {
      for (int i = lane; i < tw * th; i += 32) {
        const int r = i / tw, c = i - r * tw;
        grid[(size_t)(Y0 + r) * A.W + X0 + c] = tile[r * A.pitch + c];
      }
    }
    __syncwarp();
  }
}

__global__ void k_compose_slices(int8_t* __restrict__ grids, const uint32_t* __restrict__ maps, int n_flights,
                                 int W, int H, int S, int row0, int rows) {
  const size_t per = (size_t)W * rows;
  const size_t i = (size_t)blockIdx.x * blockDim.x + threadIdx.x;
  if (i >= per * n_flights) return;
  const int flight = (int)(i / per);
  const size_t cell = (size_t)row0 * W + (i - (size_t)flight * per);
  int8_t* g = grids + (size_t)flight * W * H + cell;
  int v = (int)*g;
  const uint32_t* m = maps + (size_t)flight * (S - 1) * W * H + cell;
  for (int s = 1; s < S; s++, m += (size_t)W * H) {
    const uint32_t w = __ldg(m);
    const int flo = (int)(int8_t)(w & 0xffu), fhi = (int)(int8_t)((w >> 8) & 0xffu), a = (int)w >> 16;
    v = min(max(v + a, flo), fhi);
  }
  *g = (int8_t)v;
}

struct Beam {
  int m;
  int n2;
  uint32_t inv;
  int sM, sN;
  int ra, rb;
  int end_delta;
  int base;
  int k0;
};

__device__ __forceinline__ Beam decode_beam(uint2 rec, uint2 org, int P, int bx0, int by0, int lo_occ, int end_nohit) {
  Beam b;
  const int dx = sext12(rec.x), dy = sext12(rec.x >> 12);
  const int adx = abs(dx), ady = abs(dy);
  const bool xmaj = adx >= ady;
  b.m = (rec.x & kRayValid) ? (xmaj ? adx : ady) : -1;
  b.n2 = 2 * (xmaj ? ady : adx);
  b.inv = rec.y;
  const bool xpos = dx >= 0, ypos = dy >= 0;
  const int sx = xpos ? 1 : -1, sy = ypos ? P : -P;
  b.sM = xmaj ? sx : sy;
  b.sN = xmaj ? sy : sx;
  if (xmaj) { b.ra = xpos ? (ypos ? 0 : 8) : 4; b.rb = (xpos == ypos) ? 1 : -1; }
  else      { b.ra = ypos ? 2 : 6;              b.rb = (xpos == ypos) ? -1 : 1; }
  b.end_delta = (rec.x & kRayHit) ? lo_occ : end_nohit;
  b.base = ((int)(org.y & 0xffffu) - by0) * P + ((int)(org.x & 0xffffu) - bx0);
  b.k0 = (int)(org.x >> 16);
  return b;
}

#ifndef UQS_UN
#define UQS_UN 3
#endif
#ifndef UQS_MINB
#define UQS_MINB 8
#endif
template <int NW, int FAN, int PROD, bool PROBE = false>
__global__ void __launch_bounds__((NW + PROD) * 32, (NW <= 4) ? (PROD ? 6 : UQS_MINB) : ((NW <= 8) ? 4 : ((NW <= 16) ? 2 : 1)))
k_replay_flights(FlightArgs A, ProbeArgs Q) {
  constexpr int NT = (NW + PROD) * 32;
  const bool producer = PROD && (threadIdx.x >> 5) == NW;
  int8_t* grid_s = reinterpret_cast<int8_t*>(uqs_smem);
  __shared__ int s_flight;
  const int lane = threadIdx.x & 31, w = threadIdx.x >> 5;
  const int P = A.pitch;
  uint8_t* ring = reinterpret_cast<uint8_t*>(uqs_smem) + (size_t)P * A.max_rows + (size_t)w * A.ring_size;
  const int ring_mask = A.ring_size - 1;
  const uint32_t grid_sa = (uint32_t)__cvta_generic_to_shared(grid_s);
  __shared__ int s_const[2];
  if (threadIdx.x == 0) { s_const[0] = A.lo_free; s_const[1] = A.lo_min; }
  __syncthreads();
  const uint32_t const_sa = (uint32_t)__cvta_generic_to_shared(s_const);
  const int lo_free = (int)lds_u32(const_sa), lo_min = (int)lds_u32(const_sa + 4u), lo_max = in_reg(A.lo_max);
  const uint32_t ring_sa = (uint32_t)__cvta_generic_to_shared(ring);
  const uint32_t dec_sa = (grid_sa + (uint32_t)(P * A.max_rows + NW * A.ring_size + 4 * NW) + 15u) & ~15u;

  for (;;) {
    if (threadIdx.x == 0) s_flight = (int)atomicAdd(A.job_counter, 1ull);
    __syncthreads();
    const int flight = s_flight;
    if (flight >= A.n_flights) break;
    const int4 box = A.boxes[flight];
    const int bx0 = box.x, by0 = box.y, bw = box.z - box.x, bh = box.w - box.y;
    const int8_t* grid_hbm = A.grids + (size_t)flight * A.W * A.H;
    int pb = 0, pe = 0, next_pf = 0x7fffffff;
    if (PROBE) {
      pb = Q.start[flight];
      pe = Q.start[flight + 1];
      if (pb < pe) next_pf = Q.probes[pb].x;
    }
    if (bw <= 0 || bh <= 0) {
      if (PROBE)
        for (int i = pb + threadIdx.x; i < pe; i += NT) { const int4 pr = Q.probes[i]; Q.values[pr.z] = (uint32_t)(int)grid_hbm[pr.y]; }
      __syncthreads();
      continue;
    }
    int8_t* grid_g = A.grids + (size_t)flight * A.W * A.H + (size_t)by0 * A.W + bx0;
    const bool vec = (((A.W | bx0 | bw) & 3) == 0) && ((reinterpret_cast<size_t>(grid_g) & 3) == 0);

    if (A.accumulate) {
      if (vec) {
        const int wpr = bw >> 2;
        for (int i = threadIdx.x; i < wpr * bh; i += NT) {
          const int r = i / wpr, c = i - r * wpr;
          reinterpret_cast<uint32_t*>(grid_s + r * P)[c] = reinterpret_cast<const uint32_t*>(grid_g + (size_t)r * A.W)[c];
        }
      } else {
        for (int i = threadIdx.x; i < bw * bh; i += NT) {
          const int r = i / bw, c = i - r * bw;
          grid_s[r * P + c] = grid_g[(size_t)r * A.W + c];
        }
      }
    } else {
      for (int i = threadIdx.x; i < ((P * bh) >> 2); i += NT) reinterpret_cast<uint32_t*>(grid_s)[i] = 0u;
    }
    __syncthreads();

    const uint4* frames = A.frames + (size_t)flight * A.n_frames;
    const uint2* rays = A.rays + (size_t)flight * A.n_frames * 32;
    const SmemRegion RG = { grid_sa, grid_sa + (uint32_t)(P * bh) };
    const SmemRegion RR = { ring_sa, ring_sa + (uint32_t)A.ring_size };
    const SmemRegion RD = { dec_sa, dec_sa + (uint32_t)((NW < kDecSlotsMax ? NW : kDecSlotsMax) * kDecSlotBytes) };
    (void)RG; (void)RR; (void)RD;
    constexpr int R = NW < kDecSlotsMax ? NW : kDecSlotsMax;
    constexpr int L = R / 2;
    auto decode_store = [&](uint2 rec, uint2 org, int slot) {
      const Beam b = decode_beam(rec, org, P, bx0, by0, A.lo_occ, A.end_nohit);
      const int mx = __reduce_max_sync(0xffffffffu, b.m);
      const uint32_t at = dec_sa + (uint32_t)slot * kDecSlotBytes;
      UQS_CHECK(at + 16u * (uint32_t)lane, 16u, RD); UQS_CHECK(at + 512u + 4u * (uint32_t)lane, 4u, RD); UQS_CHECK(at + 1024u, 16u, RD);
      sts_v4(at + 16u * (uint32_t)lane, b.inv, (uint32_t)b.n2, (uint32_t)b.m, (uint32_t)b.sM);
      sts_u32(at + 512u + 4u * (uint32_t)lane, ((uint32_t)b.sN << 16) | (b.rb < 0 ? 0x1000u : 0u) | ((uint32_t)b.ra << 8) |
                                                   ((uint32_t)b.end_delta & 0xffu));
      if (lane == 0) sts_v4(at + 1024u, (uint32_t)b.base, (uint32_t)b.k0, (uint32_t)mx, (org.y & kFrameSorted) ? 1u : 0u);
    };
    uint2 raw_rec, raw_org;
    if (PROD) {
      if (producer) {
        for (int g = 0; g < L && g < A.n_frames; g++)
          decode_store(__ldg(&rays[(size_t)g * 32 + lane]), __ldg(reinterpret_cast<const uint2*>(&frames[g])), g);
        const int g = min(L, A.n_frames - 1);
        raw_rec = __ldg(&rays[(size_t)g * 32 + lane]);
        raw_org = __ldg(reinterpret_cast<const uint2*>(&frames[g]));
      }
    } else {
      if (w < L && w < A.n_frames)
        decode_store(__ldg(&rays[(size_t)w * 32 + lane]), __ldg(reinterpret_cast<const uint2*>(&frames[w])), w);
      const int g = min(w + L, A.n_frames - 1);
      raw_rec = __ldg(&rays[(size_t)g * 32 + lane]);
      raw_org = __ldg(reinterpret_cast<const uint2*>(&frames[g]));
    }
    __syncthreads();
    for (int f = 0; f < A.n_frames; f++) {
      if (producer) {
        const int g = f + L;
        if (g < A.n_frames) decode_store(raw_rec, raw_org, g & (R - 1));
        const int gn = min(g + 1, A.n_frames - 1);
        raw_rec = __ldg(&rays[(size_t)gn * 32 + lane]);
        raw_org = __ldg(reinterpret_cast<const uint2*>(&frames[gn]));
        __syncthreads();
        continue;
      }
      const uint32_t at = dec_sa + (uint32_t)(f & (R - 1)) * kDecSlotBytes;
      UQS_CHECK(at + 16u * (uint32_t)lane, 16u, RD); UQS_CHECK(at + 1024u, 16u, RD);
      const uint4 fv = lds_v4(at + 1024u);
      uint4 dv = make_uint4(0u, 0u, 0u, 0u);
      uint32_t dw = 0u;
      if (!FAN || ((w - f - 1) & (NW - 1)) < (int)fv.y) {
        dv = lds_v4(at + 16u * (uint32_t)lane);
        dw = lds_u32(at + 512u + 4u * (uint32_t)lane);
      }
      const uint32_t inv = dv.x;
      const int n2 = (int)dv.y, m = (int)dv.z, h2 = m & ~1;
      const int sM = (int)dv.w, sN = (int)dw >> 16;
      Beam B;
      B.end_delta = (int)(signed char)(dw & 0xffu);
      B.ra = (int)((dw >> 8) & 0xfu);
      B.rb = (dw & 0x1000u) ? -1 : 1;
      B.k0 = (int)fv.y;
      const int base = (int)fv.x, mmax = (int)fv.z;
      const bool sorted = fv.w != 0u;
      const int kshared = B.k0;

      for (int k = (w - f - 1) & (NW - 1); k < kshared; k += NW) {
        const bool act = k <= m;
        const int q = minor_steps(k, n2, h2, inv);
        const int addr = base + k * sM + q * sN;
        const int delta = (k == m) ? B.end_delta : -lo_free;
        const unsigned actm0 = __ballot_sync(0xffffffffu, act);
        if (sorted && !__any_sync(0xffffffffu, act && k == m)) {
          if (actm0 == 0u) continue;
          if (actm0 == 0xffffffffu) {
            const int paddr = __shfl_up_sync(0xffffffffu, addr, 1);
            const bool head = lane == 0 || paddr != addr;
            const unsigned heads = __ballot_sync(0xffffffffu, head);
            const unsigned above_h = (heads >> 1) >> lane;
            int len = above_h ? __ffs(above_h) : 32 - lane;
            bool apply = head;
            const int a_last = __shfl_sync(0xffffffffu, addr, 31);
            if (heads != 1u && __shfl_sync(0xffffffffu, addr, 0) == a_last) {
              const int len0 = __shfl_sync(0xffffffffu, len, 0);
              if (lane == 31 - __clz(heads)) len += len0;
              if (lane == 0) apply = false;
            }
            if (apply) {
              const uint32_t cell = grid_sa + (uint32_t)addr;
              UQS_CHECK(cell, 1u, RG);
              sts_u8(cell, max(lds_s8(cell) - len * lo_free, lo_min));
            }
            __syncwarp();
            continue;
          }
          const unsigned lower = actm0 & ((1u << lane) - 1u);
          const int prev = lower ? (31 - __clz(lower)) : lane;
          const int paddr = __shfl_sync(0xffffffffu, addr, prev);
          const bool headr = act && (lower == 0u || paddr != addr);
          const unsigned heads = __ballot_sync(0xffffffffu, headr);
          const int first = __ffs(actm0) - 1, last = 31 - __clz(actm0);
          const int a_first = __shfl_sync(0xffffffffu, addr, first), a_last = __shfl_sync(0xffffffffu, addr, last);
          const unsigned above_h = heads & ~(0xffffffffu >> (31 - lane));
          const unsigned span = above_h ? ((1u << (__ffs(above_h) - 1)) - 1u) : 0xffffffffu;
          int len = __popc(actm0 & span & ~((1u << lane) - 1u));
          bool apply = headr;
          if ((heads & (heads - 1u)) != 0u && a_first == a_last) {
            const int len_first = __shfl_sync(0xffffffffu, len, first);
            if (lane == 31 - __clz(heads)) len += len_first;
            if (lane == first) apply = false;
          }
          if (apply) {
            const uint32_t cell = grid_sa + (uint32_t)addr;
            UQS_CHECK(cell, 1u, RG);
            sts_u8(cell, max(lds_s8(cell) - len * lo_free, lo_min));
          }
          __syncwarp();
          continue;
        }
        const unsigned key = act ? (unsigned)addr : (0x80000000u | (unsigned)lane);
        const unsigned prevkey = __shfl_up_sync(0xffffffffu, key, 1);
        const bool bound = lane == 0 || prevkey != key;
        const bool head = act && bound;
        int pos = B.ra * k + B.rb * q;
        if (pos == 8 * k) pos = 0;
        const int slot = pos & ring_mask;
        if (head) { UQS_CHECK(ring_sa + (uint32_t)slot, 1u, RR); sts_u8(ring_sa + (uint32_t)slot, lane); }
        __syncwarp();
        const bool lost = head && lds_s8(ring_sa + (uint32_t)slot) != lane;
        const unsigned boundm = __ballot_sync(0xffffffffu, bound);
        const unsigned actm = __ballot_sync(0xffffffffu, act);
        unsigned pend = __ballot_sync(0xffffffffu, lost);
        const uint32_t cell = grid_sa + (uint32_t)addr;
        if (act) UQS_CHECK(cell, 1u, RG);
        if ((boundm & actm) == actm && pend == 0u) {
          if (act) sts_u8(cell, min(max(lds_s8(cell) + delta, lo_min), lo_max));
        } else {
          const unsigned upto = 0xffffffffu >> (31 - lane);
          const int start = 31 - __clz(boundm & upto);
          const unsigned above = boundm & ~upto;
          const int end = above ? (__ffs(above) - 2) : 31;
          unsigned peers = (0xffffffffu >> (31 - end)) & (0xffffffffu << start);
          while (pend) {
            const int a = __shfl_sync(0xffffffffu, addr, __ffs(pend) - 1);
            const bool same = act && addr == a;
            const unsigned members = __ballot_sync(0xffffffffu, same);
            pend &= ~members;
            if (same) peers = members;
          }
          const unsigned endm = __ballot_sync(0xffffffffu, act && k == m);
          const bool uniform = (peers & endm) == 0u;
          if (act && uniform && lane == __ffs(peers) - 1) {
            sts_u8(cell, max(lds_s8(cell) - __popc(peers) * lo_free, lo_min));
          }
          const bool mixed = act && !uniform;
          const int rank = __popc(peers & ((1u << lane) - 1u));
          const int rounds = __reduce_max_sync(0xffffffffu, mixed ? rank : -1);
          for (int r = 0; r <= rounds; r++) {
            if (mixed && rank == r) sts_u8(cell, min(max(lds_s8(cell) + delta, lo_min), lo_max));
            __syncwarp();
          }
        }
        __syncwarp();
      }

      const uint32_t gbase = grid_sa + (uint32_t)base;
      const int free_delta = -lo_free;
      constexpr int UN = UQS_UN;
      if (FAN) {
        constexpr int NS = NW / 4;
        const uint32_t bq = (uint32_t)((w & 3) * 8 + (lane >> 2));
        const int j = lane & 3;
        UQS_CHECK(at + 16u * bq, 16u, RD); UQS_CHECK(at + 512u + 4u * bq, 4u, RD);
        const uint4 ev = lds_v4(at + 16u * bq);
        const uint32_t ew = lds_u32(at + 512u + 4u * bq);
        const uint32_t inv_f = ev.x;
        const int n2_f = (int)ev.y, m_f = (int)ev.z, h2_f = m_f & ~1, sM_f = (int)ev.w, sN_f = (int)ew >> 16;
        const int fmax = __reduce_max_sync(0xffffffffu, m_f);
        int kb = kshared + 4 * (w >> 2);
        int mu[UN];
#pragma unroll
        for (int u = 0; u < UN; u++) mu[u] = in_reg(m_f - j - u * 4 * NS);
        for (; kb < fmax; kb += UN * 4 * NS) {
          uint32_t addr[UN];
          int val[UN];
          bool on[UN];
#pragma unroll
          for (int u = 0; u < UN; u++) {
            const int ku = kb + j + u * 4 * NS;
            addr[u] = gbase + (uint32_t)(ku * sM_f + minor_steps(ku, n2_f, h2_f, inv_f) * sN_f);
            on[u] = kb < mu[u];
          }
#pragma unroll
          for (int u = 0; u < UN; u++) if (on[u]) { UQS_CHECK(addr[u], 1u, RG); val[u] = lds_s8(addr[u]); }
#pragma unroll
          for (int u = 0; u < UN; u++) if (on[u]) sts_u8(addr[u], __viaddmax_s32(val[u], free_delta, lo_min));
        }
        if ((w >> 2) == ((f + 1) & (NS - 1)) && j == 0 && m_f >= kshared) {
          const uint32_t cell = gbase + (uint32_t)(m_f * sM_f + (n2_f >> 1) * sN_f);
          UQS_CHECK(cell, 1u, RG);
          sts_u8(cell, min(max(lds_s8(cell) + (int)(signed char)(ew & 0xffu), lo_min), lo_max));
        }
      } else {
      int k = B.k0 + ((w - B.k0) & (NW - 1));
      int mu[UN];
#pragma unroll
      for (int u = 0; u < UN; u++) mu[u] = in_reg(m - u * NW);
      for (; k < mmax; k += UN * NW) {
        uint32_t addr[UN];
        int val[UN];
        bool on[UN];
#pragma unroll
        for (int u = 0; u < UN; u++) {
          const int ku = k + u * NW;
          addr[u] = gbase + (uint32_t)(ku * sM + minor_steps(ku, n2, h2, inv) * sN);
          on[u] = k < mu[u];
        }
#pragma unroll
        for (int u = 0; u < UN; u++) if (on[u]) { UQS_CHECK(addr[u], 1u, RG); val[u] = lds_s8(addr[u]); }
#pragma unroll
        for (int u = 0; u < UN; u++) if (on[u]) sts_u8(addr[u], __viaddmax_s32(val[u], free_delta, lo_min));
      }
      if (w == ((f + 1) & (NW - 1)) && mmax >= kshared) {
        if (m >= kshared) {
          const uint32_t cell = gbase + (uint32_t)(m * sM + (n2 >> 1) * sN);
          UQS_CHECK(cell, 1u, RG);
          sts_u8(cell, min(max(lds_s8(cell) + B.end_delta, lo_min), lo_max));
        }
      }
      }
      if (!PROD && (f & (NW - 1)) == w) {
        const int g = f + L;
        if (g < A.n_frames) decode_store(raw_rec, raw_org, g & (R - 1));
        const int gn = min(g + NW, A.n_frames - 1);
        raw_rec = __ldg(&rays[(size_t)gn * 32 + lane]);
        raw_org = __ldg(reinterpret_cast<const uint2*>(&frames[gn]));
      }
      __syncthreads();
      if (PROBE) {
        while (next_pf == f) {
          const int i = pb + (int)threadIdx.x;
          const int4 pr = i < pe ? Q.probes[i] : make_int4(-1, 0, 0, 0);
          const bool take = pr.x == f;
          if (take) {
            const int gy = pr.y / A.W, gx = pr.y - gy * A.W;
            int v;
            if (gx >= bx0 && gx < bx0 + bw && gy >= by0 && gy < by0 + bh) {
              const uint32_t cell = grid_sa + (uint32_t)((gy - by0) * P + (gx - bx0));
              UQS_CHECK(cell, 1u, RG);
              v = lds_s8(cell);
            } else {
              v = (int)grid_hbm[pr.y];
            }
            Q.values[pr.z] = (uint32_t)v;
          }
          pb += __syncthreads_count(take);
          next_pf = pb < pe ? Q.probes[pb].x : 0x7fffffff;
        }
      }
    }

    if (vec) {
      const int wpr = bw >> 2;
      for (int i = threadIdx.x; i < wpr * bh; i += NT) {
        const int r = i / wpr, c = i - r * wpr;
        reinterpret_cast<uint32_t*>(grid_g + (size_t)r * A.W)[c] = reinterpret_cast<const uint32_t*>(grid_s + r * P)[c];
      }
    } else {
      for (int i = threadIdx.x; i < bw * bh; i += NT) {
        const int r = i / bw, c = i - r * bw;
        grid_g[(size_t)r * A.W + c] = grid_s[r * P + c];
      }
    }
    __syncthreads();
  }
}

__global__ void k_flight_boxes(int n_flights, int groups_per_flight, const uint2* __restrict__ groups, int W, int H,
                               int4* __restrict__ boxes, int* __restrict__ dims) {
  const int flight = (int)((blockIdx.x * (long long)blockDim.x + threadIdx.x) >> 5);
  const int lane = threadIdx.x & 31;
  if (flight >= n_flights) return;
  int x0 = 0x7fff, x1 = -1, y0 = 0x7fff, y1 = -1;
  for (int g = lane; g < groups_per_flight; g += 32) {
    const uint2 b = __ldg(&groups[(size_t)flight * groups_per_flight + g]);
    const int bx0 = (int)(b.x & 0xffffu), bx1 = (int)(b.x >> 16), by0 = (int)(b.y & 0xffffu), by1 = (int)(b.y >> 16);
    if (bx0 <= bx1 && by0 <= by1) { x0 = min(x0, bx0); x1 = max(x1, bx1); y0 = min(y0, by0); y1 = max(y1, by1); }
  }
  x0 = __reduce_min_sync(0xffffffffu, x0); x1 = __reduce_max_sync(0xffffffffu, x1);
  y0 = __reduce_min_sync(0xffffffffu, y0); y1 = __reduce_max_sync(0xffffffffu, y1);
  if (lane == 0) {
    int4 box = make_int4(0, 0, 0, 0);
    if (x0 <= x1 && y0 <= y1) {
      x1 += 1; y1 += 1;
      if ((W & 3) == 0) { x0 &= ~3; x1 = min((x1 + 3) & ~3, W); }
      box = make_int4(x0, y0, x1, y1);
      atomicMax(&dims[0], x1 - x0);
      atomicMax(&dims[1], y1 - y0);
    }
    boxes[flight] = box;
  }
}

static void (*flight_kernel(int nw, int fan, int prod))(FlightArgs, ProbeArgs) {
  if (prod) return nw == 4 ? k_replay_flights<4, 0, 1> : (nw == 8 ? k_replay_flights<8, 0, 1> : (nw == 32 ? k_replay_flights<16, 0, 1> : k_replay_flights<16, 0, 1>));
  if (fan) return nw == 4 ? k_replay_flights<4, 1, 0> : (nw == 8 ? k_replay_flights<8, 1, 0> : (nw == 32 ? k_replay_flights<32, 1, 0> : k_replay_flights<16, 1, 0>));
  return nw == 4 ? k_replay_flights<4, 0, 0> : (nw == 8 ? k_replay_flights<8, 0, 0> : (nw == 32 ? k_replay_flights<32, 0, 0> : k_replay_flights<16, 0, 0>));
}

__global__ void k_publish_dims(const int* __restrict__ dims, volatile int* host_dims) {
  host_dims[0] = dims[0];
  host_dims[1] = dims[1];
  __threadfence_system();
}

cudaError_t flight_boxes_launch(int n_flights, int groups_per_flight, const uint2* groups, int W, int H, int4* boxes,
                                int* dims, int* host_dims_dev, cudaStream_t st) {
  k_flight_boxes<<<(unsigned)((n_flights + 3) / 4), 128, 0, st>>>(n_flights, groups_per_flight, groups, W, H, boxes, dims);
  k_publish_dims<<<1, 1, 0, st>>>(dims, host_dims_dev);
  return cudaGetLastError();
}

static int flight_threads(int nw, int prod) { return (std::min(nw, prod ? 16 : 32) + (prod ? 1 : 0)) * 32; }

cudaError_t flights_prepare(int nw, int fan, int prod, size_t smem, int* ctas_per_sm) {
  cudaError_t e = cudaFuncSetAttribute(flight_kernel(nw, fan, prod), cudaFuncAttributeMaxDynamicSharedMemorySize, (int)smem);
  if (e != cudaSuccess) return e;
  return cudaOccupancyMaxActiveBlocksPerMultiprocessor(ctas_per_sm, flight_kernel(nw, fan, prod), flight_threads(nw, prod), smem);
}

cudaError_t flights_launch(int nw, int fan, int prod, unsigned grid, size_t smem, cudaStream_t st, const FlightArgs& A) {
  flight_kernel(nw, fan, prod)<<<grid, flight_threads(nw, prod), smem, st>>>(A, ProbeArgs{});
  return cudaGetLastError();
}

static void (*flight_probe_kernel(int nw))(FlightArgs, ProbeArgs) {
  return nw == 4 ? k_replay_flights<4, 0, 0, true> : (nw == 8 ? k_replay_flights<8, 0, 0, true> : (nw == 32 ? k_replay_flights<32, 0, 0, true> : k_replay_flights<16, 0, 0, true>));
}

cudaError_t flights_probe_prepare(int nw, size_t smem, int* ctas_per_sm) {
  cudaError_t e = cudaFuncSetAttribute(flight_probe_kernel(nw), cudaFuncAttributeMaxDynamicSharedMemorySize, (int)smem);
  if (e != cudaSuccess) return e;
  return cudaOccupancyMaxActiveBlocksPerMultiprocessor(ctas_per_sm, flight_probe_kernel(nw), flight_threads(nw, 0), smem);
}

cudaError_t flights_probe_launch(int nw, unsigned grid, size_t smem, cudaStream_t st, const FlightArgs& A, const ProbeArgs& Q) {
  flight_probe_kernel(nw)<<<grid, flight_threads(nw, 0), smem, st>>>(A, Q);
  return cudaGetLastError();
}

cudaError_t tiles_prepare(bool probe, size_t smem, int* ctas_per_sm) {
  void (*k)(ReplayArgs, ProbeArgs) = probe ? k_replay_tiles<true> : k_replay_tiles<false>;
  cudaError_t e = cudaFuncSetAttribute(k, cudaFuncAttributeMaxDynamicSharedMemorySize, (int)smem);
  if (e != cudaSuccess) return e;
  return cudaOccupancyMaxActiveBlocksPerMultiprocessor(ctas_per_sm, k, kReplayThreads, smem);
}

cudaError_t tiles_launch(bool probe, unsigned grid, size_t smem, cudaStream_t st, const ReplayArgs& A, const ProbeArgs& Q) {
  if (probe) k_replay_tiles<true><<<grid, kReplayThreads, smem, st>>>(A, Q);
  else       k_replay_tiles<false><<<grid, kReplayThreads, smem, st>>>(A, Q);
  return cudaGetLastError();
}

__global__ void k_zero(unsigned char* __restrict__ p, size_t bytes) {
  const size_t head = min(bytes, (size_t)((16 - (reinterpret_cast<size_t>(p) & 15)) & 15));
  const size_t n16 = (bytes - head) >> 4;
  const size_t tid = (size_t)blockIdx.x * blockDim.x + threadIdx.x, nth = (size_t)gridDim.x * blockDim.x;
  uint4* q = reinterpret_cast<uint4*>(p + head);
  for (size_t i = tid; i < n16; i += nth) q[i] = make_uint4(0u, 0u, 0u, 0u);
  const size_t tail0 = head + (n16 << 4);
  if (tid < head) p[tid] = 0;
  if (tid < bytes - tail0) p[tail0 + tid] = 0;
}

cudaError_t zero_async(void* p, size_t bytes, cudaStream_t st) {
  if (bytes == 0) return cudaSuccess;
  const size_t want = (bytes / 16 + 255) / 256;
  const unsigned blocks = (unsigned)std::min<size_t>(std::max<size_t>(want, 1), 148 * 16);
  k_zero<<<blocks, 256, 0, st>>>(reinterpret_cast<unsigned char*>(p), bytes);
  return cudaGetLastError();
}

__global__ void __launch_bounds__(kReplayThreads)
k_rmw_peak(int tile_bytes, int iters, int lo_min, int* sink) {
  const int lane = threadIdx.x & 31, wic = threadIdx.x >> 5;
  int8_t* tile = reinterpret_cast<int8_t*>(uqs_smem) + (size_t)wic * tile_bytes;
  for (int i = lane; i < tile_bytes; i += 32) tile[i] = 0;
  __syncwarp();
  const uint32_t base = (uint32_t)__cvta_generic_to_shared(tile) + (uint32_t)lane;
  const uint32_t mask = (uint32_t)tile_bytes - 1u;
  uint32_t off = 0;
  for (int it = 0; it < iters; it++) {
    int v[8];
#pragma unroll
    for (int u = 0; u < 8; u++) v[u] = lds_s8(base + ((off + 32u * u) & mask));
#pragma unroll
    for (int u = 0; u < 8; u++) sts_u8(base + ((off + 32u * u) & mask), max(v[u] - 1, lo_min));
    off += 256u + 32u;
  }
  __syncwarp();
  if (tile[lane] == 77) *sink = 1;
}

__global__ void __launch_bounds__(kReplayThreads)
k_atoms_peak(int tile_bytes, int iters, int* sink) {
  const int lane = threadIdx.x & 31, wic = threadIdx.x >> 5;
  int* tile = reinterpret_cast<int*>(uqs_smem + (size_t)wic * tile_bytes);
  for (int i = lane; i < tile_bytes / 4; i += 32) tile[i] = 0;
  __syncwarp();
  const uint32_t mask = (uint32_t)(tile_bytes / 4) - 1u;
  uint32_t off = (uint32_t)lane;
  for (int it = 0; it < iters; it++) {
#pragma unroll
    for (int u = 0; u < 8; u++) atomicAdd(&tile[(off + 32u * u) & mask], -1);
    off += 256u + 32u;
  }
  __syncwarp();
  if (tile[lane] == 77) *sink = 1;
}

}
```

micro-quad-slam_b200/csrc/uqs_kernels.cuh:

```cuda
#pragma once
#include "uqs_device.cuh"

namespace uqs {

constexpr int kReplayThreads = 256;
constexpr int kReplayWarps = kReplayThreads / 32;
constexpr int kReplayQueueBytes = 64 * 12;
constexpr int kDecSlotBytes = 32 * 32 + 16;
constexpr int kDecSlotsMax = 4;
constexpr int kJobGroup = 64;

struct ReplayArgs {
  const uint4* frames;
  const uint2* groups;
  const uint2* rays;
  int8_t* grids;
  unsigned long long* job_counter;
  const uint32_t* tile_order;
  unsigned long long total_jobs;
  int n_flights, n_frames, groups_per_flight;
  int W, H;
  int row0, rows;
  int sw, sh, nsx, nsy;
  int pitch, tile_bytes;
  int pitch_cells;
  int slices;
  int groups_per_slice;
  uint32_t* maps;
  int lo_free, lo_occ, lo_min, lo_max, end_nohit;
  int accumulate;
};

struct FlightArgs {
  const uint4* frames;
  const uint2* rays;
  int8_t* grids;
  unsigned long long* job_counter;
  int n_flights, n_frames;
  const int4* boxes;
  int W, H, pitch;
  int max_rows;
  int ring_size;
  int lo_free, lo_occ, lo_min, lo_max, end_nohit;
  int accumulate;
};

struct ProbeArgs {
  const int4* probes;
  const int* start;
  uint32_t* values;
  int n_buckets;
};

struct ScanState;

__global__ void k_pose_increments(long long total, int n_samples, const uint32_t* t_ms,
                                  const float* rate_x, const float* rate_y, const float* h_m,
                                  const float* yaw_deg, const uint8_t* q, float deg2rad, float* inc_n,
                                  float* inc_e, unsigned long long* domain_errors);
__global__ void k_pose_chain(int n_flights, int n_samples, const float* inc_n, const float* inc_e,
                             float* xo, float* yo);
__global__ void k_pose_scan(int n_flights, int n_samples, int parts_per_flight, const float* inc_n,
                            const float* inc_e, float* xo, float* yo, volatile ScanState* state,
                            unsigned int* ticket);
int pose_scan_tile();
size_t pose_scan_state_bytes();
cudaError_t zero_async(void* p, size_t bytes, cudaStream_t st);
int pose_scan_threads();

__global__ void k_ray_setup(const __grid_constant__ DevParams p, int n_frames, const float* x,
                            const float* y, const float* yaw_deg, const float* ranges,
                            const uint8_t* kind, int want_k0, const uint32_t* inv_table, uint4* frames, uint2* groups,
                            uint2* rays,
                            unsigned long long* stats);
__global__ void k_records_to_cells(long long n_frames, const uint4* frames, const uint2* rays,
                                   int32_t* cells, int32_t* origin);
__global__ void k_sincosf(size_t n, const float* a, float* s, float* c);
__global__ void k_world_to_grid_one(DevParams p, float wx, float wy, int* out);
cudaError_t tiles_prepare(bool probe, size_t smem, int* ctas_per_sm);
cudaError_t tiles_launch(bool probe, unsigned grid, size_t smem, cudaStream_t st, const ReplayArgs& A, const ProbeArgs& Q);
__global__ void k_compose_slices(int8_t* grids, const uint32_t* maps, int n_flights, int W, int H, int S, int row0,
                                 int rows);
cudaError_t flights_probe_prepare(int nw, size_t smem, int* ctas_per_sm);
cudaError_t flights_probe_launch(int nw, unsigned grid, size_t smem, cudaStream_t st, const FlightArgs& A, const ProbeArgs& Q);
cudaError_t flight_boxes_launch(int n_flights, int groups_per_flight, const uint2* groups, int W, int H, int4* boxes,
                                int* dims, int* host_dims_dev, cudaStream_t st);
cudaError_t flights_prepare(int nw, int fan, int prod, size_t smem, int* ctas_per_sm);
cudaError_t flights_launch(int nw, int fan, int prod, unsigned grid, size_t smem, cudaStream_t st, const FlightArgs& A);
__global__ void k_rmw_peak(int tile_bytes, int iters, int lo_min, int* sink);
__global__ void k_atoms_peak(int tile_bytes, int iters, int* sink);
__global__ void k_recenter_decide_one(float res, float size_m, float ox, float oy, float x, float y, int* out);
__global__ void k_recenter_shift(const int8_t* src, int8_t* dst, int W, int H, int sx, int sy);
__global__ void k_frontier_scores(DevParams p, const int8_t* grid, int n, const float* x, const float* y,
                                  const float* yaw_deg, const float* offset_deg, int* scores,
                                  unsigned long long* domain_errors);

}
```

Measured before the change: 738.5 billion.

## Pre-encode rays in major/minor form and drop shared-memory decode slots

The ray record now stores major length, doubled minor length, axis and sign bits directly, so consumers skip the abs/compare decoding of signed 12-bit deltas. The flight replay kernel drops the shared-memory decode ring (and the producer-warp and fan-layout variants). Instead each warp reads its next record from global memory with a one-frame register prefetch and an L2 prefetch several frames ahead. This frees shared memory and removes the decode stores and reads, at the cost of per-warp global loads and recomputing step parameters in registers.

```diff
diff --git a/micro-quad-slam_b200/csrc/uqs_api.cu b/micro-quad-slam_b200/csrc/uqs_api.cu
--- a/micro-quad-slam_b200/csrc/uqs_api.cu
+++ b/micro-quad-slam_b200/csrc/uqs_api.cu
@@ -295,11 +295,10 @@
       size_t fsmem = 0;
       auto fit = [&](int w, int* ring, size_t* bytes, int* ctas) -> cudaError_t {
         *ring = 256;
-        const size_t dec_bytes = (size_t)std::min(w, kDecSlotsMax) * kDecSlotBytes + 16;
-        while (*ring > 32 && region + (size_t)(*ring + 4) * w + dec_bytes > kFlightSmemMax) *ring >>= 1;
-        *bytes = region + (size_t)(*ring + 4) * w + dec_bytes;
+        while (*ring > 32 && region + (size_t)(*ring + 4) * w > kFlightSmemMax) *ring >>= 1;
+        *bytes = region + (size_t)(*ring + 4) * w;
         *ctas = 0;
-        return *bytes <= kFlightSmemMax ? flights_prepare(w, g_ctx.flight_fan, g_ctx.flight_prod, *bytes, ctas) : cudaSuccess;
+        return *bytes <= kFlightSmemMax ? flights_prepare(w, *bytes, ctas) : cudaSuccess;
       };
       if (g_ctx.flight_warps) {
         e = fit(fnw, &ring_size, &fsmem, &f_ctas);
@@ -352,7 +351,7 @@
         }
         const unsigned fgrid = (unsigned)std::min<long long>(nf, (long long)f_ctas * g_ctx.sm_count);
         KernelTimer t_rep(2);
-        e = flights_launch(fnw, g_ctx.flight_fan, g_ctx.flight_prod, fgrid, fsmem, st, FA);
+        e = flights_launch(fnw, fgrid, fsmem, st, FA);
         t_rep.stop();
         if (e != cudaSuccess) return cuda_fail(e, "k_replay_flights launch");
         g_ctx.launches += 2;
@@ -620,7 +619,7 @@
 }
 
 int uqs_set_decode_warp(int on) {
-  g_ctx.flight_prod = on < 0 ? kDefaultDecodeWarp : (on ? 1 : 0);
+  (void)on;
   return UQS_OK;
 }
 
@@ -630,7 +629,7 @@
 }
 
 int uqs_set_fan_layout(int on) {
-  g_ctx.flight_fan = on < 0 ? kDefaultFanLayout : (on ? 1 : 0);
+  (void)on;
   return UQS_OK;
 }
 
diff --git a/micro-quad-slam_b200/csrc/uqs_device.cuh b/micro-quad-slam_b200/csrc/uqs_device.cuh
--- a/micro-quad-slam_b200/csrc/uqs_device.cuh
+++ b/micro-quad-slam_b200/csrc/uqs_device.cuh
@@ -21,8 +21,11 @@
 }
 
 constexpr int      kMaxRayCells   = 1024;
+constexpr uint32_t kRayXMajor     = 1u << 23;
 constexpr uint32_t kRayHit        = 1u << 24;
 constexpr uint32_t kRayValid      = 1u << 25;
+constexpr uint32_t kRayXNeg       = 1u << 26;
+constexpr uint32_t kRayYNeg       = 1u << 27;
 constexpr uint32_t kFrameHasOrigin = 1u << 16;
 constexpr uint32_t kFrameSorted    = 1u << 17;
 constexpr uint32_t kEmptyBoxLoHi  = 0x00007fffu;
@@ -141,7 +144,22 @@
   return 1;
 }
 
-__device__ __forceinline__ int sext12(uint32_t v) { return ((int)(v << 20)) >> 20; }
+__device__ __forceinline__ uint32_t ray_w0(int dx, int dy, bool hit) {
+  const int adx = abs(dx), ady = abs(dy);
+  const bool xmaj = adx >= ady;
+  const int m = xmaj ? adx : ady, n = xmaj ? ady : adx;
+  return (uint32_t)m | ((uint32_t)(2 * n) << 11) | (xmaj ? kRayXMajor : 0u) | (hit ? kRayHit : 0u) | kRayValid |
+         (dx < 0 ? kRayXNeg : 0u) | (dy < 0 ? kRayYNeg : 0u);
+}
+__device__ __forceinline__ int ray_m(uint32_t w0) { return (int)(w0 & 0x7ffu); }
+__device__ __forceinline__ int ray_n2(uint32_t w0) { return (int)((w0 >> 11) & 0xfffu); }
+__device__ __forceinline__ void ray_dxdy(uint32_t w0, int& dx, int& dy) {
+  const int m = ray_m(w0), n = ray_n2(w0) >> 1;
+  const bool xmaj = (w0 & kRayXMajor) != 0u;
+  const int adx = xmaj ? m : n, ady = xmaj ? n : m;
+  dx = (w0 & kRayXNeg) ? -adx : adx;
+  dy = (w0 & kRayYNeg) ? -ady : ady;
+}
 
 __device__ __forceinline__ float frontier_ray_angle(const DevParams& p, float yaw_deg, float offset_deg, int r) {
   const float ro = (r == 0) ? 0.0f : (r == 1) ? 15.0f : -15.0f;
diff --git a/micro-quad-slam_b200/csrc/uqs_host.h b/micro-quad-slam_b200/csrc/uqs_host.h
--- a/micro-quad-slam_b200/csrc/uqs_host.h
+++ b/micro-quad-slam_b200/csrc/uqs_host.h
@@ -9,8 +9,6 @@
 
 namespace uqs {
 
-constexpr int kDefaultDecodeWarp = 0;
-constexpr int kDefaultFanLayout = 0;
 
 struct DevBuf {
   void* p = nullptr;
@@ -49,8 +47,6 @@
   int flight_warps = 0;
   int k0_bias = 0;
   int pitch_mod = -1;
-  int flight_prod = kDefaultDecodeWarp;
-  int flight_fan = kDefaultFanLayout;
   int host_chunk = 0;
   bool copy_only = false;
   bool chip_shared = false;
diff --git a/micro-quad-slam_b200/csrc/uqs_kernels.cu b/micro-quad-slam_b200/csrc/uqs_kernels.cu
--- a/micro-quad-slam_b200/csrc/uqs_kernels.cu
+++ b/micro-quad-slam_b200/csrc/uqs_kernels.cu
@@ -273,18 +273,19 @@
     const int gx0 = s_org[w][0], gy0 = s_org[w][1];
     const bool have_o = gx0 >= 0;
     uint32_t w0 = 0, w1 = 0;
+    int dx = 0, dy = 0;
     if (st < 0) {
       domain = 1;
     } else if (st > 0 && have_o) {
       int gx1, gy1;
       if (world_to_grid(p, ex, ey, gx1, gy1)) {
-        const int dx = gx1 - gx0, dy = gy1 - gy0;
-        const int m = max(abs(dx), abs(dy));
+        const int ddx = gx1 - gx0, ddy = gy1 - gy0;
+        const int m = max(abs(ddx), abs(ddy));
         if (m > kMaxRayCells) {
           domain = 1;
         } else {
-          w0 = ((uint32_t)dx & 0xfffu) | (((uint32_t)dy & 0xfffu) << 12) | (hit ? kRayHit : 0u) |
-               kRayValid;
+          dx = ddx; dy = ddy;
+          w0 = ray_w0(dx, dy, hit);
           w1 = __ldg(&inv_table[m]);
           xmin = min(gx0, gx1); xmax = max(gx0, gx1);
           ymin = min(gy0, gy1); ymax = max(gy0, gy1);
@@ -299,7 +300,6 @@
     int k0 = 0;
     bool frame_sorted = false;
     if (want_k0) {
-      const int dx = sext12(w0), dy = sext12(w0 >> 12);
       const int adx = abs(dx), ady = abs(dy);
       const bool xmaj = adx >= ady;
       const int m = accepted ? (xmaj ? adx : ady) : -1;
@@ -399,8 +399,10 @@
   const uint2 r = rays[i];
   int cx = -1, cy = -1;
   if (r.x & kRayValid) {
-    cx = (int)(fr.x & 0xffffu) + sext12(r.x);
-    cy = (int)(fr.y & 0xffffu) + sext12(r.x >> 12);
+    int dx, dy;
+    ray_dxdy(r.x, dx, dy);
+    cx = (int)(fr.x & 0xffffu) + dx;
+    cy = (int)(fr.y & 0xffffu) + dy;
   }
   cells[2 * i] = cx;
   cells[2 * i + 1] = cy;
@@ -505,11 +507,9 @@
     const uint32_t w0 = lds_u32(at), org = lds_u32(at + 8u * kQueueEntries);
     inv_l = lds_u32(at + 4u * kQueueEntries);
     const int gx0 = (int)(org & 0xffffu), gy0 = (int)(org >> 16);
-    const int dx = sext12(w0), dy = sext12(w0 >> 12);
-    const int adx = abs(dx), ady = abs(dy);
-    const bool xmaj = adx >= ady;
-    const int m = xmaj ? adx : ady, n = xmaj ? ady : adx, h = m >> 1;
-    const bool majpos = (xmaj ? dx : dy) >= 0, minpos = (xmaj ? dy : dx) >= 0;
+    const bool xmaj = (w0 & kRayXMajor) != 0u, xpos = (w0 & kRayXNeg) == 0u, ypos = (w0 & kRayYNeg) == 0u;
+    const int m = ray_m(w0), n2 = ray_n2(w0), n = n2 >> 1, h = m >> 1;
+    const bool majpos = xmaj ? xpos : ypos, minpos = xmaj ? ypos : xpos;
     const int c0 = xmaj ? gx0 : gy0, c1 = xmaj ? gy0 : gx0;
     const int A0 = xmaj ? X0 : Y0, A1 = xmaj ? X1 : Y1;
     const int B0 = xmaj ? Y0 : X0, B1 = xmaj ? Y1 : X1;
@@ -527,7 +527,7 @@
     const int pitch = A.pitch;
     const int cK = majpos ? (xmaj ? 1 : pitch) : (xmaj ? -1 : -pitch);
     const int cQ = minpos ? (xmaj ? pitch : 1) : (xmaj ? -pitch : -1);
-    p1 = (uint32_t)(2 * n) | ((uint32_t)m << 16);
+    p1 = (uint32_t)n2 | ((uint32_t)m << 16);
     p2 = ((uint32_t)cK & 0xffffu) | ((uint32_t)cQ << 16);
     p3 = (uint32_t)ka | ((uint32_t)kb << 11) | ((w0 & kRayHit) ? (1u << 22) : 0u);
     p4 = tile + ((uint32_t)((gy0 - Y0) * pitch + (gx0 - X0)) << (MAP ? 2 : 0));
@@ -703,7 +703,9 @@
           if (PROBE) serve(f0 + fi);
           const int gx0 = (int)(__shfl_sync(0xffffffffu, fr.x, fi) & 0xffffu);
           const int gy0 = (int)(__shfl_sync(0xffffffffu, fr.y, fi) & 0xffffu);
-          const int ex = gx0 + sext12(rec.x), ey = gy0 + sext12(rec.x >> 12);
+          int dx, dy;
+          ray_dxdy(rec.x, dx, dy);
+          const int ex = gx0 + dx, ey = gy0 + dy;
           const bool near = (rec.x & kRayValid) != 0u && min(gx0, ex) < X1 && max(gx0, ex) >= X0 && min(gy0, ey) < Y1 &&
                             max(gy0, ey) >= Y0;
           const unsigned nm = __ballot_sync(0xffffffffu, near);
@@ -765,48 +767,18 @@
   *g = (int8_t)v;
 }
 
-struct Beam {
-  int m;
-  int n2;
-  uint32_t inv;
-  int sM, sN;
-  int ra, rb;
-  int end_delta;
-  int base;
-  int k0;
-};
-
-__device__ __forceinline__ Beam decode_beam(uint2 rec, uint2 org, int P, int bx0, int by0, int lo_occ, int end_nohit) {
-  Beam b;
-  const int dx = sext12(rec.x), dy = sext12(rec.x >> 12);
-  const int adx = abs(dx), ady = abs(dy);
-  const bool xmaj = adx >= ady;
-  b.m = (rec.x & kRayValid) ? (xmaj ? adx : ady) : -1;
-  b.n2 = 2 * (xmaj ? ady : adx);
-  b.inv = rec.y;
-  const bool xpos = dx >= 0, ypos = dy >= 0;
-  const int sx = xpos ? 1 : -1, sy = ypos ? P : -P;
-  b.sM = xmaj ? sx : sy;
-  b.sN = xmaj ? sy : sx;
-  if (xmaj) { b.ra = xpos ? (ypos ? 0 : 8) : 4; b.rb = (xpos == ypos) ? 1 : -1; }
-  else      { b.ra = ypos ? 2 : 6;              b.rb = (xpos == ypos) ? -1 : 1; }
-  b.end_delta = (rec.x & kRayHit) ? lo_occ : end_nohit;
-  b.base = ((int)(org.y & 0xffffu) - by0) * P + ((int)(org.x & 0xffffu) - bx0);
-  b.k0 = (int)(org.x >> 16);
-  return b;
-}
-
 #ifndef UQS_UN
 #define UQS_UN 3
 #endif
 #ifndef UQS_MINB
 #define UQS_MINB 8
 #endif
-template <int NW, int FAN, int PROD, bool PROBE = false>
-__global__ void __launch_bounds__((NW + PROD) * 32, (NW <= 4) ? (PROD ? 6 : UQS_MINB) : ((NW <= 8) ? 4 : ((NW <= 16) ? 2 : 1)))
+constexpr int kRecPrefetch = 8;
+__device__ __forceinline__ void prefetch_l2(const void* p) { asm volatile("prefetch.global.L2 [%0];" ::"l"(p)); }
+template <int NW, bool PROBE = false>
+__global__ void __launch_bounds__(NW * 32, (NW <= 4) ? UQS_MINB : ((NW <= 8) ? 4 : ((NW <= 16) ? 2 : 1)))
 k_replay_flights(FlightArgs A, ProbeArgs Q) {
-  constexpr int NT = (NW + PROD) * 32;
-  const bool producer = PROD && (threadIdx.x >> 5) == NW;
+  constexpr int NT = NW * 32;
   int8_t* grid_s = reinterpret_cast<int8_t*>(uqs_smem);
   __shared__ int s_flight;
   const int lane = threadIdx.x & 31, w = threadIdx.x >> 5;
@@ -820,7 +792,7 @@
   const uint32_t const_sa = (uint32_t)__cvta_generic_to_shared(s_const);
   const int lo_free = (int)lds_u32(const_sa), lo_min = (int)lds_u32(const_sa + 4u), lo_max = in_reg(A.lo_max);
   const uint32_t ring_sa = (uint32_t)__cvta_generic_to_shared(ring);
-  const uint32_t dec_sa = (grid_sa + (uint32_t)(P * A.max_rows + NW * A.ring_size + 4 * NW) + 15u) & ~15u;
+  const int lo_occ = A.lo_occ, end_nohit = A.end_nohit;
 
   for (;;) {
     if (threadIdx.x == 0) s_flight = (int)atomicAdd(A.job_counter, 1ull);
@@ -867,73 +839,34 @@
     const uint2* rays = A.rays + (size_t)flight * A.n_frames * 32;
     const SmemRegion RG = { grid_sa, grid_sa + (uint32_t)(P * bh) };
     const SmemRegion RR = { ring_sa, ring_sa + (uint32_t)A.ring_size };
-    const SmemRegion RD = { dec_sa, dec_sa + (uint32_t)((NW < kDecSlotsMax ? NW : kDecSlotsMax) * kDecSlotBytes) };
-    (void)RG; (void)RR; (void)RD;
-    constexpr int R = NW < kDecSlotsMax ? NW : kDecSlotsMax;
-    constexpr int L = R / 2;
-    auto decode_store = [&](uint2 rec, uint2 org, int slot) {
-      const Beam b = decode_beam(rec, org, P, bx0, by0, A.lo_occ, A.end_nohit);
-      const int mx = __reduce_max_sync(0xffffffffu, b.m);
-      const uint32_t at = dec_sa + (uint32_t)slot * kDecSlotBytes;
-      UQS_CHECK(at + 16u * (uint32_t)lane, 16u, RD); UQS_CHECK(at + 512u + 4u * (uint32_t)lane, 4u, RD); UQS_CHECK(at + 1024u, 16u, RD);
-      sts_v4(at + 16u * (uint32_t)lane, b.inv, (uint32_t)b.n2, (uint32_t)b.m, (uint32_t)b.sM);
-      sts_u32(at + 512u + 4u * (uint32_t)lane, ((uint32_t)b.sN << 16) | (b.rb < 0 ? 0x1000u : 0u) | ((uint32_t)b.ra << 8) |
-                                                   ((uint32_t)b.end_delta & 0xffu));
-      if (lane == 0) sts_v4(at + 1024u, (uint32_t)b.base, (uint32_t)b.k0, (uint32_t)mx, (org.y & kFrameSorted) ? 1u : 0u);
-    };
-    uint2 raw_rec, raw_org;
-    if (PROD) {
-      if (producer) {
-        for (int g = 0; g < L && g < A.n_frames; g++)
-          decode_store(__ldg(&rays[(size_t)g * 32 + lane]), __ldg(reinterpret_cast<const uint2*>(&frames[g])), g);
-        const int g = min(L, A.n_frames - 1);
-        raw_rec = __ldg(&rays[(size_t)g * 32 + lane]);
-        raw_org = __ldg(reinterpret_cast<const uint2*>(&frames[g]));
-      }
-    } else {
-      if (w < L && w < A.n_frames)
-        decode_store(__ldg(&rays[(size_t)w * 32 + lane]), __ldg(reinterpret_cast<const uint2*>(&frames[w])), w);
-      const int g = min(w + L, A.n_frames - 1);
-      raw_rec = __ldg(&rays[(size_t)g * 32 + lane]);
-      raw_org = __ldg(reinterpret_cast<const uint2*>(&frames[g]));
-    }
-    __syncthreads();
+    (void)RG; (void)RR;
+    uint2 rec = __ldg(&rays[lane]);
+    uint2 org = __ldg(reinterpret_cast<const uint2*>(&frames[0]));
     for (int f = 0; f < A.n_frames; f++) {
-      if (producer) {
-        const int g = f + L;
-        if (g < A.n_frames) decode_store(raw_rec, raw_org, g & (R - 1));
-        const int gn = min(g + 1, A.n_frames - 1);
-        raw_rec = __ldg(&rays[(size_t)gn * 32 + lane]);
-        raw_org = __ldg(reinterpret_cast<const uint2*>(&frames[gn]));
-        __syncthreads();
-        continue;
-      }
-      const uint32_t at = dec_sa + (uint32_t)(f & (R - 1)) * kDecSlotBytes;
-      UQS_CHECK(at + 16u * (uint32_t)lane, 16u, RD); UQS_CHECK(at + 1024u, 16u, RD);
-      const uint4 fv = lds_v4(at + 1024u);
-      uint4 dv = make_uint4(0u, 0u, 0u, 0u);
-      uint32_t dw = 0u;
-      if (!FAN || ((w - f - 1) & (NW - 1)) < (int)fv.y) {
-        dv = lds_v4(at + 16u * (uint32_t)lane);
-        dw = lds_u32(at + 512u + 4u * (uint32_t)lane);
-      }
-      const uint32_t inv = dv.x;
-      const int n2 = (int)dv.y, m = (int)dv.z, h2 = m & ~1;
-      const int sM = (int)dv.w, sN = (int)dw >> 16;
-      Beam B;
-      B.end_delta = (int)(signed char)(dw & 0xffu);
-      B.ra = (int)((dw >> 8) & 0xfu);
-      B.rb = (dw & 0x1000u) ? -1 : 1;
-      B.k0 = (int)fv.y;
-      const int base = (int)fv.x, mmax = (int)fv.z;
-      const bool sorted = fv.w != 0u;
-      const int kshared = B.k0;
+      const uint32_t w0 = rec.x, inv = rec.y, ox = org.x, oy = org.y;
+      {
+        const int g = min(f + 1, A.n_frames - 1);
+        rec = __ldg(&rays[(size_t)g * 32 + lane]);
+        org = __ldg(reinterpret_cast<const uint2*>(&frames[g]));
+        const int gp = min(f + kRecPrefetch, A.n_frames - 1);
+        prefetch_l2(&rays[(size_t)gp * 32 + lane]);
+        prefetch_l2(&frames[gp]);
+      }
+      const bool xmaj = (w0 & kRayXMajor) != 0u, xpos = (w0 & kRayXNeg) == 0u, ypos = (w0 & kRayYNeg) == 0u;
+      const int m = (w0 & kRayValid) ? ray_m(w0) : -1, n2 = ray_n2(w0), h2 = m & ~1;
+      const int sx = xpos ? 1 : -1, sy = ypos ? P : -P;
+      const int sM = xmaj ? sx : sy, sN = xmaj ? sy : sx;
+      const int end_delta = (w0 & kRayHit) ? lo_occ : end_nohit;
+      const int base = ((int)(oy & 0xffffu) - by0) * P + ((int)(ox & 0xffffu) - bx0);
+      const int kshared = (int)(ox >> 16);
+      const bool sorted = (oy & kFrameSorted) != 0u;
+      const int mmax = __reduce_max_sync(0xffffffffu, m);
 
       for (int k = (w - f - 1) & (NW - 1); k < kshared; k += NW) {
         const bool act = k <= m;
         const int q = minor_steps(k, n2, h2, inv);
         const int addr = base + k * sM + q * sN;
-        const int delta = (k == m) ? B.end_delta : -lo_free;
+        const int delta = (k == m) ? end_delta : -lo_free;
         const unsigned actm0 = __ballot_sync(0xffffffffu, act);
         if (sorted && !__any_sync(0xffffffffu, act && k == m)) {
           if (actm0 == 0u) continue;
@@ -986,7 +919,9 @@
         const unsigned prevkey = __shfl_up_sync(0xffffffffu, key, 1);
         const bool bound = lane == 0 || prevkey != key;
         const bool head = act && bound;
-        int pos = B.ra * k + B.rb * q;
+        const int ra = xmaj ? (xpos ? (ypos ? 0 : 8) : 4) : (ypos ? 2 : 6);
+        const bool rneg = xmaj ? (xpos != ypos) : (xpos == ypos);
+        int pos = ra * k + (rneg ? -q : q);
         if (pos == 8 * k) pos = 0;
         const int slot = pos & ring_mask;
         if (head) { UQS_CHECK(ring_sa + (uint32_t)slot, 1u, RR); sts_u8(ring_sa + (uint32_t)slot, lane); }
@@ -1031,42 +966,7 @@
       const uint32_t gbase = grid_sa + (uint32_t)base;
       const int free_delta = -lo_free;
       constexpr int UN = UQS_UN;
-      if (FAN) {
-        constexpr int NS = NW / 4;
-        const uint32_t bq = (uint32_t)((w & 3) * 8 + (lane >> 2));
-        const int j = lane & 3;
-        UQS_CHECK(at + 16u * bq, 16u, RD); UQS_CHECK(at + 512u + 4u * bq, 4u, RD);
-        const uint4 ev = lds_v4(at + 16u * bq);
-        const uint32_t ew = lds_u32(at + 512u + 4u * bq);
-        const uint32_t inv_f = ev.x;
-        const int n2_f = (int)ev.y, m_f = (int)ev.z, h2_f = m_f & ~1, sM_f = (int)ev.w, sN_f = (int)ew >> 16;
-        const int fmax = __reduce_max_sync(0xffffffffu, m_f);
-        int kb = kshared + 4 * (w >> 2);
-        int mu[UN];
-#pragma unroll
-        for (int u = 0; u < UN; u++) mu[u] = in_reg(m_f - j - u * 4 * NS);
-        for (; kb < fmax; kb += UN * 4 * NS) {
-          uint32_t addr[UN];
-          int val[UN];
-          bool on[UN];
-#pragma unroll
-          for (int u = 0; u < UN; u++) {
-            const int ku = kb + j + u * 4 * NS;
-            addr[u] = gbase + (uint32_t)(ku * sM_f + minor_steps(ku, n2_f, h2_f, inv_f) * sN_f);
-            on[u] = kb < mu[u];
-          }
-#pragma unroll
-          for (int u = 0; u < UN; u++) if (on[u]) { UQS_CHECK(addr[u], 1u, RG); val[u] = lds_s8(addr[u]); }
-#pragma unroll
-          for (int u = 0; u < UN; u++) if (on[u]) sts_u8(addr[u], __viaddmax_s32(val[u], free_delta, lo_min));
-        }
-        if ((w >> 2) == ((f + 1) & (NS - 1)) && j == 0 && m_f >= kshared) {
-          const uint32_t cell = gbase + (uint32_t)(m_f * sM_f + (n2_f >> 1) * sN_f);
-          UQS_CHECK(cell, 1u, RG);
-          sts_u8(cell, min(max(lds_s8(cell) + (int)(signed char)(ew & 0xffu), lo_min), lo_max));
-        }
-      } else {
-      int k = B.k0 + ((w - B.k0) & (NW - 1));
+      int k = kshared + ((w - kshared) & (NW - 1));
       int mu[UN];
 #pragma unroll
       for (int u = 0; u < UN; u++) mu[u] = in_reg(m - u * NW);
@@ -1089,16 +989,8 @@
         if (m >= kshared) {
           const uint32_t cell = gbase + (uint32_t)(m * sM + (n2 >> 1) * sN);
           UQS_CHECK(cell, 1u, RG);
-          sts_u8(cell, min(max(lds_s8(cell) + B.end_delta, lo_min), lo_max));
-        }
-      }
-      }
-      if (!PROD && (f & (NW - 1)) == w) {
-        const int g = f + L;
-        if (g < A.n_frames) decode_store(raw_rec, raw_org, g & (R - 1));
-        const int gn = min(g + NW, A.n_frames - 1);
-        raw_rec = __ldg(&rays[(size_t)gn * 32 + lane]);
-        raw_org = __ldg(reinterpret_cast<const uint2*>(&frames[gn]));
+          sts_u8(cell, min(max(lds_s8(cell) + end_delta, lo_min), lo_max));
+        }
       }
       __syncthreads();
       if (PROBE) {
@@ -1166,10 +1058,8 @@
   }
 }
 
-static void (*flight_kernel(int nw, int fan, int prod))(FlightArgs, ProbeArgs) {
-  if (prod) return nw == 4 ? k_replay_flights<4, 0, 1> : (nw == 8 ? k_replay_flights<8, 0, 1> : (nw == 32 ? k_replay_flights<16, 0, 1> : k_replay_flights<16, 0, 1>));
-  if (fan) return nw == 4 ? k_replay_flights<4, 1, 0> : (nw == 8 ? k_replay_flights<8, 1, 0> : (nw == 32 ? k_replay_flights<32, 1, 0> : k_replay_flights<16, 1, 0>));
-  return nw == 4 ? k_replay_flights<4, 0, 0> : (nw == 8 ? k_replay_flights<8, 0, 0> : (nw == 32 ? k_replay_flights<32, 0, 0> : k_replay_flights<16, 0, 0>));
+static void (*flight_kernel(int nw))(FlightArgs, ProbeArgs) {
+  return nw == 4 ? k_replay_flights<4> : (nw == 8 ? k_replay_flights<8> : (nw == 32 ? k_replay_flights<32> : k_replay_flights<16>));
 }
 
 __global__ void k_publish_dims(const int* __restrict__ dims, volatile int* host_dims) {
@@ -1185,31 +1075,29 @@
   return cudaGetLastError();
 }
 
-static int flight_threads(int nw, int prod) { return (std::min(nw, prod ? 16 : 32) + (prod ? 1 : 0)) * 32; }
-
-cudaError_t flights_prepare(int nw, int fan, int prod, size_t smem, int* ctas_per_sm) {
-  cudaError_t e = cudaFuncSetAttribute(flight_kernel(nw, fan, prod), cudaFuncAttributeMaxDynamicSharedMemorySize, (int)smem);
+cudaError_t flights_prepare(int nw, size_t smem, int* ctas_per_sm) {
+  cudaError_t e = cudaFuncSetAttribute(flight_kernel(nw), cudaFuncAttributeMaxDynamicSharedMemorySize, (int)smem);
   if (e != cudaSuccess) return e;
-  return cudaOccupancyMaxActiveBlocksPerMultiprocessor(ctas_per_sm, flight_kernel(nw, fan, prod), flight_threads(nw, prod), smem);
-}
-
-cudaError_t flights_launch(int nw, int fan, int prod, unsigned grid, size_t smem, cudaStream_t st, const FlightArgs& A) {
-  flight_kernel(nw, fan, prod)<<<grid, flight_threads(nw, prod), smem, st>>>(A, ProbeArgs{});
+  return cudaOccupancyMaxActiveBlocksPerMultiprocessor(ctas_per_sm, flight_kernel(nw), nw * 32, smem);
+}
+
+cudaError_t flights_launch(int nw, unsigned grid, size_t smem, cudaStream_t st, const FlightArgs& A) {
+  flight_kernel(nw)<<<grid, nw * 32, smem, st>>>(A, ProbeArgs{});
   return cudaGetLastError();
 }
 
 static void (*flight_probe_kernel(int nw))(FlightArgs, ProbeArgs) {
-  return nw == 4 ? k_replay_flights<4, 0, 0, true> : (nw == 8 ? k_replay_flights<8, 0, 0, true> : (nw == 32 ? k_replay_flights<32, 0, 0, true> : k_replay_flights<16, 0, 0, true>));
+  return nw == 4 ? k_replay_flights<4, true> : (nw == 8 ? k_replay_flights<8, true> : (nw == 32 ? k_replay_flights<32, true> : k_replay_flights<16, true>));
 }
 
 cudaError_t flights_probe_prepare(int nw, size_t smem, int* ctas_per_sm) {
   cudaError_t e = cudaFuncSetAttribute(flight_probe_kernel(nw), cudaFuncAttributeMaxDynamicSharedMemorySize, (int)smem);
   if (e != cudaSuccess) return e;
-  return cudaOccupancyMaxActiveBlocksPerMultiprocessor(ctas_per_sm, flight_probe_kernel(nw), flight_threads(nw, 0), smem);
+  return cudaOccupancyMaxActiveBlocksPerMultiprocessor(ctas_per_sm, flight_probe_kernel(nw), nw * 32, smem);
 }
 
 cudaError_t flights_probe_launch(int nw, unsigned grid, size_t smem, cudaStream_t st, const FlightArgs& A, const ProbeArgs& Q) {
-  flight_probe_kernel(nw)<<<grid, flight_threads(nw, 0), smem, st>>>(A, Q);
+  flight_probe_kernel(nw)<<<grid, nw * 32, smem, st>>>(A, Q);
   return cudaGetLastError();
 }
 
diff --git a/micro-quad-slam_b200/csrc/uqs_kernels.cuh b/micro-quad-slam_b200/csrc/uqs_kernels.cuh
--- a/micro-quad-slam_b200/csrc/uqs_kernels.cuh
+++ b/micro-quad-slam_b200/csrc/uqs_kernels.cuh
@@ -6,8 +6,6 @@
 constexpr int kReplayThreads = 256;
 constexpr int kReplayWarps = kReplayThreads / 32;
 constexpr int kReplayQueueBytes = 64 * 12;
-constexpr int kDecSlotBytes = 32 * 32 + 16;
-constexpr int kDecSlotsMax = 4;
 constexpr int kJobGroup = 64;
 
 struct ReplayArgs {
@@ -85,8 +83,8 @@
 cudaError_t flights_probe_launch(int nw, unsigned grid, size_t smem, cudaStream_t st, const FlightArgs& A, const ProbeArgs& Q);
 cudaError_t flight_boxes_launch(int n_flights, int groups_per_flight, const uint2* groups, int W, int H, int4* boxes,
                                 int* dims, int* host_dims_dev, cudaStream_t st);
-cudaError_t flights_prepare(int nw, int fan, int prod, size_t smem, int* ctas_per_sm);
-cudaError_t flights_launch(int nw, int fan, int prod, unsigned grid, size_t smem, cudaStream_t st, const FlightArgs& A);
+cudaError_t flights_prepare(int nw, size_t smem, int* ctas_per_sm);
+cudaError_t flights_launch(int nw, unsigned grid, size_t smem, cudaStream_t st, const FlightArgs& A);
 __global__ void k_rmw_peak(int tile_bytes, int iters, int lo_min, int* sink);
 __global__ void k_atoms_peak(int tile_bytes, int iters, int* sink);
 __global__ void k_recenter_decide_one(float res, float size_m, float ox, float oy, float x, float y, int* out);
```

New measurement: 691.7 billion (median of 6 runs). 6.3% lower.
